# initc3/HoneyBadgerMPC

Measured on AMD Instinct MI355X. Metric: shares reconstructed/sec (batch open, n=64 t=21), higher is better.
Workload: dtype u256 (integer mod p): exact int8 x int8 -> int32 byte-split GEMM on the matrix cores; the high half of every sum folded mod p on the matrix cores too, one-word Barrett quotient

## Files before the change

### honeybadgermpc_amd/_capi.py

```python
import ctypes
import os

import numpy as np

_HERE = os.path.dirname(os.path.abspath(__file__))
LIB_PATH = os.environ.get("HBMPC_HIP_LIB") or os.path.join(_HERE, "lib", "libhbmpc_hip.so")

HB_OK, HB_ERR_SINGULAR, HB_ERR_BAD_ARG, HB_ERR_UNSUPPORTED = 0, 1, 2, 3
HB_ERR_NO_DEVICE, HB_ERR_HIP, HB_ERR_MISMATCH, HB_ERR_RETRY = 4, 5, 6, 7
HB_DEC_COLLECTING, HB_DEC_DONE, HB_DEC_DISAGREE, HB_DEC_UNSUPPORTED, HB_DEC_PENDING = 0, 1, 2, 3, 4
HB_DEC_OPT_DEFER, HB_DEC_OPT_BESIDE = 1, 2
HB_EW_ADD, HB_EW_SUB, HB_EW_MUL, HB_EW_NEG = 0, 1, 2, 3
HB_EW_SELFTEST_BEAVER, HB_EW_SELFTEST_INV, HB_EW_SELFTEST_BROADCAST = 4, 5, 0x100
HB_PM_AUTO, HB_PM_DIRECT, HB_PM_NTT = 0, 1, 2
HB_PM_SELFTEST_SUMS, HB_PM_SELFTEST_POWERS, HB_PM_SELFTEST_TABLES, HB_PM_SELFTEST_MAC, HB_PM_SELFTEST_CONV = 0, 1, 2, 3, 4
HB_BF_SELFTEST_MASK, HB_BF_SELFTEST_SWITCH, HB_BF_SELFTEST_INDEX, HB_BF_SELFTEST_HALVE = 0, 1, 2, 3
HB_MIMC_SUB, HB_MIMC_PAIR = 1, 2
HB_MIMC_SELFTEST_PLAIN, HB_MIMC_SELFTEST_ROUND, HB_MIMC_SELFTEST_FIRST = 0, 1, 2
HB_JJ_SCALAR_BROADCAST, HB_JJ_POINT_BROADCAST = 1, 2
HB_JJ_SELFTEST_SCALAR_MUL, HB_JJ_SELFTEST_DOUBLE_TABLE, HB_JJ_SELFTEST_MASK, HB_JJ_SELFTEST_STAGE1 = 0, 1, 2, 3
HB_JJ_SELFTEST_STAGE2, HB_JJ_SELFTEST_STAGE3, HB_JJ_SELFTEST_SCALE = 4, 5, 6
HB_FXP_MOD, HB_FXP_TRUNC, HB_FXP_NEG_TRUNC = 0, 1, 2
HB_FXP_SELFTEST_MASK, HB_FXP_SELFTEST_TRUNC_PR, HB_FXP_SELFTEST_LEAVES = 0, 1, 2
HB_FXP_SELFTEST_CARRY_MASK, HB_FXP_SELFTEST_CARRY_COMBINE, HB_FXP_SELFTEST_FINISH = 3, 4, 5
# ... 101 lines not shown
    "hb_lt_dmask": (_i, [_vp, _vp, _vp, _vp, _vp, _vp, _i, _vp, _vp, _vp, _vp, _vp, _vp, _i64, _vp]),
    "hb_lt_mid": (_i, [_vp, _vp, _vp, _vp, _i, _vp, _vp, _vp, _vp, _vp, _vp, _vp, _vp, _vp, _vp, _vp, _i64, _vp]),
    "hb_lt_xor_finish": (_i, [_vp, _vp, _vp, _vp, _vp, _vp, _vp, _vp, _i64, _vp]),
    "hb_off_mul_add": (_i, [_vp, _vp, _vp, _vp, _vp, _i64, _vp]),
    "hb_off_invsqrt_scale": (_i, [_vp, _vp, _vp, _i, _vp, _i64, _vp, _vp]),
    "hb_off_degree_check": (_i, [_vp, _vp, _i, _i64, _i, _vp, _vp]),
    "hb_mat_mul": (_i, [_vp, _vp, _vp, _vp, _i, _vp, _i64, _i, _i, _i, _vp]),
    "hb_mat_constants": (_i, [_i, _vp]),
    "hb_quick_interp_check": (_i, [_vp, _vp, _i, _vp, _i, _vp, _i, _vp, _i64, _i64, _i64, _vp, _vp, _vp]),
    "hb_quick_interp_check_map": (_i, [_vp, _vp, _i, _vp, _i, _vp, _i, _vp, _i64, _i64, _i64, _vp, _vp, _vp, _vp]),
    "hb_quick_dec_create": (_i, [_vp, _vp, _i, _pp, _vp]),
    "hb_quick_dec_arrivals": (_i, [_vp, _vp, _i, _i, _i, _vp]),
    "hb_quick_dec_decide": (_i, [_vp, _vp, _i, _vp, _i64, _i64, _i64, _vp, _vp, _vp, _vp]),
    "hb_quick_dec_launch": (_i, [_vp, _vp, _i, _vp, _i64, _i64, _i64, _vp, _vp]),
    "hb_quick_dec_verdict": (_i, [_vp, _vp, _vp]),
    "hb_quick_dec_beside": (_i, [_vp, _i]),
    "hb_quick_dec_destroy": (None, [_vp]),
    "hb_dec_create": (_i, [_vp, _vp, _i, _i, _i, _pp, _vp]),
    "hb_dec_begin": (_i, [_vp, _vp, _i64, _i, _vp, _vp, _i, _vp]),
    "hb_dec_arrived1": (_i, [_vp, _i]),
    "hb_dec_options": (_i, [_vp, _i]),
    "hb_dec_settle": (_i, [_vp]),
    "hb_dec_arrived": (_i, [_vp, _vp, _i, _vp, _vp]),
    "hb_dec_verdict": (_i, [_vp, _vp, _vp]),
    "hb_dec_arrivals_list": (_i, [_vp, _vp, _i, _vp]),
    "hb_dec_destroy": (None, [_vp]),
    "hb_wait_create": (_i, [_vp, _i, _pp]),
    "hb_wait_begin": (_i, [_vp, _vp, _i64, _i64, _i, _i, _i, _i, _vp, _vp, _vp]),
    "hb_wait_arrived1": (_i, [_vp, _i, _i]),
    "hb_wait_result": (_i, [_vp, _i, _vp, _vp, _i, _vp]),
    "hb_wait_destroy": (None, [_vp]),
    "hb_symbols_fetch": (_i, [_vp, _vp, _i, _i64, _i64, _vp, _i, _vp, _vp]),
    "hb_candidate_check": (_i, [_vp, _vp, _i, _vp, _i, _vp, _i64, _i64, _vp, _vp, _vp]),
    "hb_stream_after": (_i, [_vp, _vp, _vp]),
    "hb_side_stream": (_i, [_vp, _pp]),
    "hb_probe_create": (_i, [_vp, _vp, _i, _i, _pp, _vp]),
    "hb_probe_feed": (_i, [_vp, _vp, _i, _vp, _i64, _i64, _i, _vp, _vp, _vp]),
    "hb_probe_reset": (_i, [_vp]),
    "hb_probe_workgroups": (_i, [_vp, _i]),
    "hb_probe_points_fed": (_i, [_vp]),
    "hb_probe_destroy": (None, [_vp]),
    "hb_matvec": (_i, [_vp, _vp, _vp, HbView, _vp, _vp, HbView, _i64, _vp]),
    "hb_matvec_check": (_i, [_vp, _vp, _vp, HbView, _vp, _vp, HbView, _vp, _i, _vp, _i64, _vp]),
    "hb_vandermonde_batch_evaluate": (_i, [_vp, _vp, _i, _vp, _i64, _i, _vp, _vp]),
    "hb_vandermonde_batch_interpolate": (_i, [_vp, _vp, _i, _vp, _i64, _vp, _vp]),
    "hb_fft_batch_evaluate": (_i, [_vp, _vp, _i, _vp, _i64, _i, _i, _vp, _vp]),
    "hb_fft_batch_interpolate": (_i, [_vp, _vp, _i, _vp, _i, _vp, _i64, _vp, _vp]),
    "hb_gao_decode": (_i, [_vp, _vp, _i, _i, _vp, _i64, _vp, _vp, _vp, _vp, _vp]),
    "hb_wb_decode": (_i, [_vp, _vp, _i, _i, _vp, _vp, _i64, _vp, _vp, _vp, _vp]),
    "hb_sqrt_mod": (_i, [_vp, _vp, _i64, _vp, _vp, _vp]),
    "hb_open_plan_create": (_i, [_vp, _i, _i, _i, _vp, _vp, _i, _vp, _vp, _i, _i64, _pp, _vp]),
    "hb_open_r1_encode": (_i, [_vp, _vp, _i64, _vp, _vp]),
    "hb_open_r1_decode": (_i, [_vp, _vp, _i64, _vp, _vp]),
    "hb_open_r2_decode": (_i, [_vp, _vp, _i64, _vp, _vp]),
    "hb_open_status": (_i, [_vp, _vp]),
    "hb_open_plan_set_option": (_i, [_vp, _i, _i]),
    "hb_open_plan_get_option": (_i, [_vp, _i, _vp]),
    "hb_open_plan_destroy": (None, [_vp]),
    "hb_selftest_mulmod": (_i, [_vp, _i, _vp, _vp, _vp]),
    "hb_selftest_ew": (_i, [_vp, _i, _i, _vp, _vp, _i64]),
    "hb_selftest_pm": (_i, [_vp, _i, _i, _vp, _vp, _i64, _i, _i64, _vp]),
    "hb_selftest_bf": (_i, [_vp, _i, _i, _vp, _i64, _i, _vp]),
    "hb_selftest_mimc": (_i, [_vp, _i, _i, _vp, _vp, _i, _i, _i64, _vp, _i64]),
    "hb_selftest_jj": (_i, [_vp, _i, _i, _vp, _vp, _vp, _i, _i64, _vp, _i64]),
    "hb_selftest_fxp": (_i, [_vp, _i, _i, _vp, _vp, _vp, _i64]),
    "hb_selftest_bd": (_i, [_vp, _i, _i, _vp, _vp, _vp, _i64]),
    "hb_selftest_div": (_i, [_vp, _i, _i, _vp, _vp, _vp, _i64]),
    "hb_selftest_eq": (_i, [_vp, _i, _i, _vp, _vp, _vp, _i64]),
    "hb_selftest_lt": (_i, [_vp, _i, _i, _vp, _vp, _vp, _i64]),
    "hb_selftest_off": (_i, [_vp, _i, _i, _vp, _vp, _i64]),
    "hb_selftest_rf": (_i, [_vp, _i, _i, _vp, _vp, _vp]),
    "hb_selftest_mat": (_i, [_vp, _i, _i, _vp, _vp, _vp]),
}
DEBUG_SYMBOLS = {
    "hb_debug_mm8_create": (_i, [_vp, _vp, _i, _i, _pp]),
    "hb_debug_mm8_apply": (_i, [_vp, _vp, _vp, _i64, _i64, _i64, _vp, _i64, _i64, _i64, _i64, _vp, _vp]),
    "hb_debug_occupancy": (_i, [_i, _i, _vp, _vp]),
    "hb_debug_reload_env": (None, []),
    "hb_debug_pm_slab_bytes": (None, [_i64]),
    "hb_debug_rf_stats": (None, [_vp]),
    "hb_debug_rf_profile": (None, [_i]),
    "hb_debug_mat_split": (None, [_i]),
    "hb_debug_matvec_route": (_i, [_vp, _vp, _i64, _vp]),
}

_lib = None


def load_library():
    global _lib
    if _lib is not None:
        return _lib
    import torch

    if torch.cuda.is_available():
        torch.cuda.init()
    if not os.path.exists(LIB_PATH):
        raise HbmpcBackendError(
            f"{LIB_PATH} not found: build it with honeybadgermpc_amd/csrc/build.sh "
            "(or __graft_entry__.build()).  There is no CPU fallback."
        )
    try:
        lib = ctypes.CDLL(LIB_PATH)
    except OSError as e:
        raise HbmpcBackendError(f"cannot load {LIB_PATH}: {e}") from e
    for name, (restype, argtypes) in list(SYMBOLS.items()) + list(DEBUG_SYMBOLS.items()):
        fn = getattr(lib, name)
        fn.restype = restype
        fn.argtypes = argtypes
    _lib = lib
    if _marshal is not None and hasattr(_marshal, "bind_dec"):
        _marshal.bind_dec(ctypes.cast(lib.hb_dec_arrived1, ctypes.c_void_p).value)
        if hasattr(_marshal, "bind_wait"):
            _marshal.bind_wait(ctypes.cast(lib.hb_wait_arrived1, ctypes.c_void_p).value)
    return lib


def _load_marshal():
    try:
        import importlib.util

        path = os.path.join(_HERE, "lib", "_hbmarshal.so")
        spec = importlib.util.spec_from_file_location("_hbmarshal", path)
        mod = importlib.util.module_from_spec(spec)
        spec.loader.exec_module(mod)
        return mod
    except Exception:
        return None


_marshal = _load_marshal()


def ints_to_limbs(values, modulus, nbytes=32):
    if _marshal is not None:
        raw = _marshal.pack(values, modulus, nbytes)
        return np.frombuffer(bytearray(raw), dtype=np.uint64).reshape(len(values), nbytes // 8)
    buf = bytearray(len(values) * nbytes)
    off = 0
    for v in values:
        if v < 0:
            raise OverflowError("can't convert negative int to unsigned")
        if v >= modulus:
            v %= modulus
        buf[off : off + nbytes] = v.to_bytes(nbytes, "little")
        off += nbytes
    return np.frombuffer(buf, dtype=np.uint64).reshape(len(values), nbytes // 8)


def limbs_to_ints(arr, nbytes=32):
    if _marshal is not None:
        return _marshal.unpack(np.ascontiguousarray(arr), nbytes)
    b = np.ascontiguousarray(arr).tobytes()
    return [int.from_bytes(b[i : i + nbytes], "little") for i in range(0, len(b), nbytes)]


def np_ptr(a):
    return a.ctypes.data_as(ctypes.c_void_p)


class Context:

    _cache = {}
    _seen = {}

    @classmethod
# ... 107 lines not shown
```

### honeybadgermpc_amd/csrc/gen_mm8.py

```python
#!/usr/bin/env python3
import os

NC = 47
MAXKB = 4
XB = 180
ABUF = [[196, 200], [204, 208]]
F_SETS = [212, 234]
F_KMIN = -2
CLOBBER_LO, CLOBBER_HI = 180, 255
HALF_RHOS = [(0, 1), (2, 3)]


def f(s, k, e):
    assert -2 <= k <= 8 and e in (0, 1)
    return F_SETS[s] + 2 * (k - F_KMIN) + e


def windows(rho):
    return [q for q in range(-2, 8) if -7 <= 4 * q + rho <= 31]


def cols_of(rho):
    return sorted({4 * q + rho + 7 + 8 * g for q in windows(rho) for g in (0, 1)})


def half_columns(half):
    return sorted(c for rho in HALF_RHOS[half] for c in cols_of(rho))


def lds_loads(kb, xs_op, as_op):
    a0, a1 = ABUF[kb & 1]
    out = []
    for e in (0, 1):
        for h in (0, 1):
            out.append(f"ds_read_b128 v[{XB + 8 * e + 4 * h}:{XB + 8 * e + 4 * h + 3}], {xs_op} offset:{((kb * 2 + e) * 2 + h) * 1024}")
    out.append(f"ds_read_b128 v[{a0}:{a0 + 3}], {as_op} offset:{(kb * 2) * 1024}")
    out.append(f"ds_read_b128 v[{a1}:{a1 + 3}], {as_op} offset:{(kb * 2 + 1) * 1024}")
    return out


def interleave(mfmas, ops):
    out = []
    if not mfmas:
        return list(ops)
    n = len(mfmas)
    per = (len(ops) + max(n - 1, 1) - 1) // max(n - 1, 1)
    pi = 0
    for i, m in enumerate(mfmas):
        if i == n - 1:
            out += ops[pi:]
            pi = len(ops)
        out.append(m)
        if i < n - 1:
            out += ops[pi:pi + per]
            pi += per
    return out


def asm_half(half, nkb, skip=False):
    assert not skip or nkb >= 2
    cols = half_columns(half)
    pos = {c: i for i, c in enumerate(cols)}
    ncol = len(cols)
    xs_op, as_op, bias = f"%{ncol}", f"%{ncol + 1}", f"%{ncol + 2}"
    L = []
    for s in range(2):
        for k in (-2, 8):
            for e in (0, 1):
                L.append(f"v_mov_b32 v{f(s, k, e)}, 0")
    L += lds_loads(0, xs_op, as_op)[:(5 if skip else 6)]
    groups = [(kb, rho) for kb in range(nkb) for rho in HALF_RHOS[half]]

    def prep(gi):
        kb, rho = groups[gi]
        s = gi & 1
        ops = []
        if rho == HALF_RHOS[half][0]:
            ops.append("s_waitcnt lgkmcnt(0)")
            for e in (0, 1):
                for k in range(8):
                    ops.append(f"v_xor_b32 v{f(s, k, e)}, 0x80808080, v{XB + 8 * e + k}")
                ops.append(f"v_mov_b32 v{f(s, -1, e)}, 0")
            if rho != 0:
                for e in (0, 1):
                    for k in range(-1, 8):
                        ops.append(f"v_alignbyte_b32 v{f(s, k, e)}, v{f(s, k + 1, e)}, v{f(s, k, e)}, {rho}")
        else:
            for e in (0, 1):
                for k in range(-1, 8):
                    ops.append(f"v_alignbyte_b32 v{f(s, k, e)}, v{f(1 - s, k + 1, e)}, v{f(1 - s, k, e)}, 1")
        return ops

    started = set()

    def mfmas(gi):
        kb, rho = groups[gi]
        s = gi & 1
        out = []
        for q in windows(rho):
            r = f(s, q, 0)
            assert r % 2 == 0
            for grp in (0, 1):
                if skip and kb == 0 and grp == 1:
                    continue
                c = 4 * q + rho + 7 + 8 * grp
                ab = ABUF[kb & 1][grp]
                cin = f"%{pos[c]}"
                if c not in started:
                    assert kb == 0 or (skip and kb == 1)
                    cin = bias
                    started.add(c)
                out.append(f"v_mfma_i32_16x16x64_i8 %{pos[c]}, v[{ab}:{ab + 3}], v[{r}:{r + 3}], {cin}")
        return out

    L += prep(0) + ["s_nop 1"]
    for gi in range(len(groups)):
        nxt = gi + 1 < len(groups)
        kb, rho = groups[gi]
        if rho == HALF_RHOS[half][0] and kb + 1 < nkb:
            L += lds_loads(kb + 1, xs_op, as_op)
        L += interleave(mfmas(gi), prep(gi + 1) if nxt else [])
        if nxt:
            L.append("s_nop 0")
    assert started == set(cols)
    L += ["s_nop 7", "s_nop 7"]
    return L, ncol


def emit():
    out = ["// GENERATED by gen_mm8.py -- do not edit", ""]
    out.append("// column held by accumulator i of each half (half 0: rho in {0,1}; half 1: rho in {2,3})")
    for half in range(2):
        cols = half_columns(half)
        out.append(f"// half {half}: {cols}")
    assert half_columns(0) == [c for c in range(NC) if c % 4 in (0, 3)] and half_columns(1) == [c for c in range(NC) if c % 4 in (1, 2)]
    out.append("template <int NKB, int HALF, bool SKIP = false> struct Mm8Phase;")
    clob = ", ".join(f'"v{r}"' for r in range(CLOBBER_LO, CLOBBER_HI + 1))
    for nkb, skip in [(k, False) for k in range(1, MAXKB + 1)] + [(k, True) for k in range(2, MAXKB + 1)]:
        for half in range(2):
            lines, ncol = asm_half(half, nkb, skip)
            out.append(f"template <> struct Mm8Phase<{nkb}, {half}, {'true' if skip else 'false'}> {{")
            out.append("    static __device__ __forceinline__ void run(v4i (&acc)[24], uint32_t xs_addr, uint32_t as_addr, v4i biasv) {")
            out.append("        asm volatile(")
            for ln in lines:
                out.append(f'            "{ln}\\n\\t"')
            outs = ", ".join(f'"=&v"(acc[{i}])' for i in range(ncol))
            out.append(f"            : {outs}")
            out.append('            : "v"(xs_addr), "v"(as_addr), "v"(biasv)')
            out.append(f'            : {clob}, "memory");')
            out.append("    }")
            out.append("};")
    return "\n".join(out) + "\n"


if __name__ == "__main__":
    here = os.path.dirname(os.path.abspath(__file__))
    text = emit()
    path = os.path.join(here, "hb_mm8_body.inc")
    old = open(path).read() if os.path.exists(path) else None
    if old != text:
        open(path, "w").write(text)
    print(path)
```

### honeybadgermpc_amd/csrc/hb_common.hpp

```cpp
#pragma once
#include <hip/hip_runtime.h>
#include <stdint.h>
#include <stdio.h>
#include <string.h>

#include <functional>
#include <map>
#include <mutex>
#include <string>
#include <vector>

#include "../../include/hbmpc_hip.h"
#include "fp29.hpp"

namespace hb {
struct FastMatrix;
struct Mm8Matrix;
struct Mm8wMatrix;
}
namespace hb {

struct Wide { static constexpr int NL = 9, NW = 8; };
struct Narrow { static constexpr int NL = 3, NW = 2; };

constexpr int OT = 4;

template <int NL, int NW>
__device__ __forceinline__ void eval_at_point_128(uint32_t (&r)[NL], const uint32_t *__restrict__ x_packed, const uint32_t *__restrict__ poly, int d,
                                                  const FpParams<NL> &P, uint32_t (*red)[NL]) {
    const int tid = threadIdx.x;
    uint32_t xd[NL], xm[NL], acc[NL];
    load_digits<NL, NW>(xd, x_packed);
    to_mont(xm, xd, P);
#pragma unroll
    for (int q = 0; q < NL; q++) acc[q] = 0;
    for (int l = tid; l < d; l += 128) {
        uint32_t pw[NL], cd[NL], m[NL];
        fp_pow_u32(pw, xm, (uint32_t)l, P);
        load_digits<NL, NW>(cd, poly + (size_t)l * NW);
        mont_mul(m, cd, pw, P);
        fp_add(acc, acc, m, P);
    }
#pragma unroll
    for (int q = 0; q < NL; q++) red[tid][q] = acc[q];
    __syncthreads();
    for (int w = 64; w >= 1; w >>= 1) {
        if (tid < w) {
            uint32_t a[NL], b[NL], t[NL];
#pragma unroll
            for (int q = 0; q < NL; q++) { a[q] = red[tid][q]; b[q] = red[tid + w][q]; }
            fp_add(t, a, b, P);
#pragma unroll
            for (int q = 0; q < NL; q++) red[tid][q] = t[q];
        }
        __syncthreads();
    }
#pragma unroll
    for (int q = 0; q < NL; q++) r[q] = red[0][q];
}

__host__ __device__ inline size_t m_index(int i, int l, int n_in, int nl, int q) {
    return (((size_t)((i / OT) * n_in + l) * (size_t)nl + (size_t)q) * OT) + (size_t)(i % OT);
}
inline int m_tiles(int n_out) { return (n_out + OT - 1) / OT; }

}

struct hb_matrix {
    hb_ctx *ctx;
    int n_out, n_in;
    uint32_t *dev;
    size_t words;
    bool cached;
    int refs;
    hb::Mm8wMatrix *wide;
    bool wide_tried;
};

namespace hb {
struct TlsError {
    static std::string &slot() { static thread_local std::string s; return s; }
    TlsError &operator=(const std::string &m) { slot() = m; return *this; }
    TlsError &operator=(const char *m) { slot() = m ? m : ""; return *this; }
    const char *c_str() const { return slot().c_str(); }
    void clear() { slot().clear(); }
    bool empty() const { return slot().empty(); }
};
struct PrescaleParams {
    uint32_t pbar[9];
    uint32_t pneg[8];
    uint32_t m0, m1;
};
}
namespace hb {
enum EnvHook {
    ENV_CACHE_CAP,
    ENV_GAO_PAIR,
    ENV_MM8W_FLAT,
    ENV_MM8W_RQ,
    ENV_MM8W_TILE16,
    ENV_MM8_NO_SKIP,
    ENV_NO_EVAL_FEW,
    ENV_NO_FUSED_SMALL,
    ENV_NO_FUSED_VALIDATE,
    ENV_NO_MFMA,
    ENV_NO_MFMA_DECODE,
    ENV_NO_MFMA_WIDE,
    ENV_NO_NARROW_FAST,
    ENV_NO_QUICK,
    ENV_NO_QUICK_PLAN,
    ENV_NTT_STAGE_LOOP,
    ENV_PROBE_WGS,
    ENV_QUICK_NO_CAND,
    ENV_UPLOAD_MODE,
    ENV_WB_NO_GAO,
    ENV_WB_NO_UNIFORM,
    ENV_COUNT
};
const char *env_hook(EnvHook h);
void env_reload();
}
struct hb_ctx {
    int device;
    int n_limbs;
    hb::FpParams<9> pw;
    hb::FpParams<3> pn;
    uint64_t p_limbs[4];
    std::recursive_mutex mu;
    int api_depth = 0;
    hb::TlsError err;
    std::map<std::string, hb_matrix *> mcache;
    std::map<std::vector<int32_t>, int32_t *> icache;
    std::map<std::string, void *> dcache;
    std::map<std::string, hb::FastMatrix *> fcache;
    std::map<std::string, hb::Mm8Matrix *> m8cache;
    struct CacheSlot { uint64_t tick; bool pinned; std::function<void()> drop; };
    std::map<std::string, CacheSlot> lru;
    uint64_t lru_clock = 0;
    size_t cache_cap = 192;
    int32_t *flag_dev;
    hb::PrescaleParams psc;
    int psc_state = 0;
    std::map<std::string, void *> ptcache;
    struct QuickSlot { void *buf = nullptr; size_t cap = 0; void *ev = nullptr; };
    std::vector<QuickSlot> qslots;
    unsigned qnext = 0;
    std::vector<void *> probe_pool, probe_host_pool;
    void *side_stream = nullptr;
    std::map<std::string, std::pair<void *, size_t>> scratch;
    void *fetch_host = nullptr, *fetch_dev = nullptr;
    int fetch_seq = 0;
    void *cand_host = nullptr, *cand_dev = nullptr;
    int32_t *cand_ticket = nullptr;
    int cand_seq = 0;
    void *after_event = nullptr;
    std::map<int, void *> wide_shared;
    std::map<std::string, std::vector<int>> wide_shapes;
    void *mm8_shared = nullptr;
    int elem_words() const { return n_limbs == 4 ? 8 : 2; }
    int nl() const { return n_limbs == 4 ? 9 : 3; }
};

struct hb_api_guard {
    hb_ctx *c;
    explicit hb_api_guard(hb_ctx *ctx) : c(ctx) { if (c) { c->mu.lock(); c->api_depth++; } }
    ~hb_api_guard() { if (c) { c->api_depth--; c->mu.unlock(); } }
    hb_api_guard(const hb_api_guard &) = delete;
    hb_api_guard &operator=(const hb_api_guard &) = delete;
};
#define HB_API_GUARD(ctxexpr) hb_api_guard hb_api_guard__(ctxexpr)

inline int ctx_scratch(hb_ctx *ctx, const char *slot, size_t bytes, void **out) {
    auto &e = ctx->scratch[slot];
    if (e.second < bytes || !e.first) {
        if (e.first) { (void)hipFree(e.first); e.first = nullptr; e.second = 0; }
        const size_t want = bytes ? bytes : 4;
        const hipError_t err = hipMalloc(&e.first, want);
        if (err != hipSuccess) { e.first = nullptr; ctx->err = std::string("scratch ") + slot + ": " + hipGetErrorString(err); return HB_ERR_HIP; }
        e.second = want;
    }
    *out = e.first;
    return HB_OK;
}
inline void ctx_scratch_free(hb_ctx *ctx) {
    for (auto &kv : ctx->scratch) if (kv.second.first) (void)hipFree(kv.second.first);
// ... 85 lines not shown
                   int64_t C, hipStream_t s, int check_skip = 0, const uint32_t *K_override = nullptr);

int launch_decode_check(hb_ctx *ctx, const FastMatrix *dec, const FastMatrix *enc, const uint32_t *cols, hb_view cv,
                        const int32_t *z_dev, uint32_t *pk_dst, hb_view pv, int64_t pk_count, int pk_rows, uint32_t *coef_dg,
                        const int32_t *mask_dev, int32_t *mismatch_dev, int64_t C, hipStream_t s, int check_skip);

bool prescale_params(hb_ctx *ctx);
int mm8_from_fast(hb_ctx *ctx, const FastMatrix *f, Mm8Matrix **out, hipStream_t s, const int32_t *rows = nullptr, int n_rows = 0);
void mm8_free(Mm8Matrix *m);
int launch_mm8(hb_ctx *ctx, const Mm8Matrix *m, const uint32_t *in, hb_view iv, const int32_t *in_rows_dev, int64_t in_count,
               uint32_t *out, hb_view ov, int64_t out_count, const int32_t *check_mask_dev, int32_t *mismatch_dev,
               int64_t C, hipStream_t s, uint32_t *copy_dst = nullptr, hb_view cpv = hb_view{0, 0}, int64_t copy_count = 0,
               int copy_rows = 0, const int32_t *check_rows_dev = nullptr);

int mm8w_from_host(hb_ctx *ctx, const uint64_t *m_host, int n_out, int n_in, Mm8wMatrix **out, hipStream_t s);
void mm8w_free(Mm8wMatrix *m);
int mm8w_route(hb_ctx *ctx, const Mm8wMatrix *m, int64_t C, int32_t *out);
int launch_mm8w(hb_ctx *ctx, const Mm8wMatrix *m, const uint32_t *in, hb_view iv, const int32_t *in_rows_dev, int64_t in_count,
                uint32_t *out, hb_view ov, int64_t out_count, const int32_t *check_mask_dev, int32_t *mismatch_dev,
                int64_t C, hipStream_t s, const uint32_t *cmp = nullptr, hb_view cv = hb_view{0, 0}, int n_store = 0);
bool fold_tables(hb_ctx *ctx, int n_bytes, uint8_t *fold, uint32_t *top8, uint32_t *mu, uint32_t *shift8);
struct FsVerdict { unsigned long long word; unsigned long long pad; };
struct FsDone { int32_t *counter; FsVerdict *host; int32_t seq; };
constexpr int32_t FS_VERDICT_NONE = 0x3fffffff;
#ifdef __HIPCC__
__device__ __forceinline__ void fs_publish_verdict(int32_t *mismatch, int32_t *first_bad, int32_t *counter, FsVerdict *host, int32_t seq) {
    const int32_t fl = mismatch ? __hip_atomic_load(mismatch, __ATOMIC_RELAXED, __HIP_MEMORY_SCOPE_AGENT) : 0;
    const int32_t fb = first_bad ? __hip_atomic_load(first_bad, __ATOMIC_RELAXED, __HIP_MEMORY_SCOPE_AGENT) : INT32_MAX;
    const uint32_t low = ((fl & 1) ? 0x80000000u : 0u) | ((fl & 0x40000000) ? 0x40000000u : 0u) | (uint32_t)((fb < 0 || fb > FS_VERDICT_NONE) ? FS_VERDICT_NONE : fb);
    __hip_atomic_store(&host->word, ((unsigned long long)(uint32_t)seq << 32) | low, __ATOMIC_RELAXED, __HIP_MEMORY_SCOPE_SYSTEM);
    if (mismatch) __hip_atomic_store(mismatch, 0, __ATOMIC_RELAXED, __HIP_MEMORY_SCOPE_AGENT);
    if (first_bad) __hip_atomic_store(first_bad, INT32_MAX, __ATOMIC_RELAXED, __HIP_MEMORY_SCOPE_AGENT);
    if (counter) __hip_atomic_store(counter, 0, __ATOMIC_RELAXED, __HIP_MEMORY_SCOPE_AGENT);
}
__device__ __forceinline__ void fs_workgroup_done(const FsDone &done, int32_t *mismatch, int32_t *first_bad) {
    if (!done.counter) return;
    asm volatile("s_waitcnt vmcnt(0)" ::: "memory");
    __syncthreads();
    if (threadIdx.x == 0 && atomicAdd(done.counter, 1) == (int)gridDim.x - 1) fs_publish_verdict(mismatch, first_bad, done.counter, done.host, done.seq);
}
#endif
inline bool fs_verdict_is(const FsVerdict *host, int32_t seq) { return (int32_t)(*reinterpret_cast<const volatile unsigned long long *>(&host->word) >> 32) == seq; }
inline void fs_verdict_read(const FsVerdict *host, int32_t *flag, int32_t *first) {
    const uint32_t low = (uint32_t)*reinterpret_cast<const volatile unsigned long long *>(&host->word);
    *flag = ((low >> 31) ? 1 : 0) | ((low & 0x40000000u) ? 0x40000000 : 0);
    const int32_t f = (int32_t)(low & 0x3fffffffu);
    *first = f == FS_VERDICT_NONE ? INT32_MAX : f;
}
struct Mm8wShared { uint32_t bias; uint32_t c80r[9], biasmod[9]; void *wp; uint32_t *zero; };
int mm8w_geometry(int n_out, int d, int *tile_rows, int *n_rt, int *nkb, size_t *a8_bytes, size_t *crow_words);
int mm8w_shared(hb_ctx *ctx, int d, const Mm8wShared **out, hipStream_t s);
void mm8w_shared_free(hb_ctx *ctx);
int launch_mm8w_raw(hb_ctx *ctx, int n_out, int d, int tile_rows, const void *a8, const uint32_t *crow, const Mm8wShared *sh,
                    const uint32_t *in, hb_view iv, const int32_t *in_rows_dev, int64_t in_count, uint32_t *out, hb_view ov, int64_t out_count,
                    const int32_t *check_mask_dev, int32_t *mismatch_dev, int64_t C, hipStream_t s, const uint32_t *cmp, hb_view cv, int n_store,
                    int32_t *first_bad_dev, uint32_t *bad_map_dev = nullptr, const FsDone *done = nullptr);
void point_tables_free(hb_ctx *ctx);
void mm8_shared_free(hb_ctx *ctx);
struct PointTable {
    int n, S;
    uint32_t *xm, *inv, *pw;
    bool usable;
    int refs;
    bool small;
    std::vector<uint16_t> xs;
    uint16_t *xs_dev;
};
int point_table(hb_ctx *ctx, const uint64_t *x_host, int n, PointTable **out, hipStream_t s);
struct QuickLayout {
    int n, d, nc, n_coef, n_out, tile_rows, nkb;
    size_t o_a8, o_crow, o_wj, o_full, o_nraw, o_mcan, o_z, o_map, o_sync, need;
    size_t o_cand, o_cand_crow;
};
int quick_layout(hb_ctx *ctx, int n, int d, int nc, int n_coef, QuickLayout *L);
int quick_build(hb_ctx *ctx, const uint64_t *x_host, const int32_t *z, const int32_t *zc, const QuickLayout &L, uint8_t *base, const Mm8wShared **shared, hipStream_t s,
                int flags = 3 );
int quick_layout_cand(hb_ctx *ctx, QuickLayout *L);
int quick_launch(hb_ctx *ctx, const QuickLayout &L, const uint8_t *base, const Mm8wShared *sh, const uint32_t *cols, hb_view cv, uint32_t *out, hb_view ov,
                 int64_t out_count, int n_store, int32_t *mismatch_dev, int32_t *first_bad_dev, int64_t C, hipStream_t s, uint32_t *bad_map_dev = nullptr,
                 const FsDone *done = nullptr);
struct FsLayout {
    int n, d, nc, n_coef, n_out, n_rt, nkb;
    size_t o_a8, o_crow, o_kt, o_mode, o_z, o_cand, o_cand_crow, need;
};
constexpr int FS_BUILD_Z = 1, FS_BUILD_ZC = 2;
int fs_layout(hb_ctx *ctx, const PointTable *pt, int d, int nc, int n_coef, FsLayout *L);
int fs_build(hb_ctx *ctx, const PointTable *pt, const int32_t *z, const int32_t *zc, const FsLayout &L, uint8_t *base, int flags, int32_t *status_dev, hipStream_t s);
int fs_launch(hb_ctx *ctx, const FsLayout &L, const uint8_t *base, const uint32_t *cols, hb_view cv, uint32_t *out, hb_view ov, int64_t out_count,
              int32_t *mismatch_dev, int32_t *first_bad_dev, uint32_t *bad_map_dev, int64_t C, hipStream_t s, const FsDone *done = nullptr,
              const int32_t *pick_zc = nullptr);
int fs_build_cand(hb_ctx *ctx, PointTable *pt, const int32_t *z, const FsLayout &L, uint8_t *base, int32_t *status_dev, hipStream_t s, bool with_z = false);
struct Mv64Matrix;
int points_on_device(hb_ctx *ctx, const uint64_t *x_host, int n, uint32_t **out, hipStream_t s);
bool mv64_applies(const hb_ctx *ctx, int d);
bool mv64_matrix_cores(const hb_ctx *ctx, int d);
int mv64_from_host(hb_ctx *ctx, const uint64_t *m_host, int n_out, int d, const int32_t *mode_host, Mv64Matrix **out, hipStream_t s);
void mv64_free(Mv64Matrix *m);
int launch_mv64(hb_ctx *ctx, const Mv64Matrix *m, const uint64_t *in, hb_view iv, const int32_t *in_rows_dev, int64_t in_count, uint64_t *out, hb_view ov,
                int64_t out_count, int32_t *mismatch_dev, int32_t *first_bad_dev, int64_t C, hipStream_t s);
int mv64_plan_tables(hb_ctx *ctx, const uint64_t *x, int n, int d, const int32_t *z, const int32_t *zc, int nc, std::vector<uint64_t> &V, std::vector<uint64_t> &Vinv,
                     std::vector<uint64_t> &P);
int quick_dec_supported(hb_quick_dec *qd, int d, int nc, int n_coef);
const Mm8wMatrix *matrix_wide(hb_ctx *ctx, const hb_matrix *m, hipStream_t s);

#define HB_DISPATCH(ctx, EXPR_W, EXPR_N)                                                          \
    do {                                                                                          \
        if ((ctx)->n_limbs == 4) { EXPR_W; } else { EXPR_N; }                                     \
    } while (0)

}
```

### honeybadgermpc_amd/csrc/hb_core.hip

```cpp
#include <algorithm>

#include <mutex>
#include <string>

#include "hb_common.hpp"

using namespace hb;

namespace {

struct U320 { uint64_t l[5]; };
inline bool ge(const U320 &a, const U320 &b) {
    for (int i = 4; i >= 0; i--) if (a.l[i] != b.l[i]) return a.l[i] > b.l[i];
    return true;
}
inline void sub(U320 &a, const U320 &b) {
    unsigned __int128 br = 0;
    for (int i = 0; i < 5; i++) {
        unsigned __int128 d = (unsigned __int128)a.l[i] - b.l[i] - (uint64_t)br;
        a.l[i] = (uint64_t)d; br = (d >> 64) & 1;
    }
}
inline void dbl_mod(U320 &a, const U320 &p) {
    for (int i = 4; i > 0; i--) a.l[i] = (a.l[i] << 1) | (a.l[i - 1] >> 63);
// ... 342 lines not shown
    return HB_OK;
}

int alloc_matrix(hb_ctx *ctx, int n_out, int n_in, hb_matrix **out) {
    hb_matrix *m = new hb_matrix();
    m->ctx = ctx; m->n_out = n_out; m->n_in = n_in; m->cached = false; m->refs = 1; m->wide = nullptr; m->wide_tried = false;
    m->words = (size_t)m_tiles(n_out) * (size_t)n_in * OT * (size_t)ctx->nl();
    if (m->words == 0) m->words = 1;
    hipError_t e = hipMalloc(&m->dev, m->words * sizeof(uint32_t));
    if (e != hipSuccess) { delete m; ctx->err = std::string("hipMalloc: ") + hipGetErrorString(e); return HB_ERR_HIP; }
    *out = m;
    return HB_OK;
}

__global__ void k_upload_copy(const uint4 *__restrict__ src, uint4 *__restrict__ dst, size_t n16) {
    const size_t i = (size_t)blockIdx.x * blockDim.x + threadIdx.x;
    if (i < n16) dst[i] = src[i];
}
int upload_table(hb_ctx *ctx, void *dst_dev, const void *src_host, size_t bytes, hipStream_t s) {
    if (bytes == 0) return HB_OK;
    static const int legacy = [] { const char *e = env_hook(ENV_UPLOAD_MODE); return e && !strcmp(e, "memcpy") ? 1 : 0; }();
    if (legacy) {
        hipError_t e = hipMemcpyAsync(dst_dev, src_host, bytes, hipMemcpyHostToDevice, s);
        if (e == hipSuccess) e = hipStreamSynchronize(s);
        if (e != hipSuccess) { ctx->err = std::string("table upload: ") + hipGetErrorString(e); return HB_ERR_HIP; }
        return HB_OK;
    }
    const size_t n16 = (bytes + 15) / 16;
    void *stage = nullptr;
    HB_HIP(ctx, hipMalloc(&stage, n16 * 16));
    hipError_t e = hipMemcpy(stage, src_host, bytes, hipMemcpyHostToDevice);
    if (e == hipSuccess) {
        if (bytes % 16 == 0) k_upload_copy<<<(unsigned)((n16 + 255) / 256), 256, 0, s>>>((const uint4 *)stage, (uint4 *)dst_dev, n16);
        else e = hipMemcpyAsync(dst_dev, stage, bytes, hipMemcpyDeviceToDevice, s);
    }
    if (e == hipSuccess) e = hipGetLastError();
    if (e == hipSuccess) e = hipStreamSynchronize(s);
    (void)hipFree(stage);
    if (e != hipSuccess) { ctx->err = std::string("table upload: ") + hipGetErrorString(e); return HB_ERR_HIP; }
    return HB_OK;
}

int upload_elems(hb_ctx *ctx, const uint64_t *host, size_t count, uint32_t **dev, hipStream_t s) {
    size_t bytes = count * (size_t)ctx->elem_words() * 4;
    HB_HIP(ctx, hipMalloc(dev, bytes ? bytes : 4));
    const int rc = upload_table(ctx, *dev, host, bytes, s);
    if (rc) { (void)hipFree(*dev); *dev = nullptr; }
    return rc;
}

int points_on_device(hb_ctx *ctx, const uint64_t *x_host, int n, uint32_t **out, hipStream_t s) {
    std::string key = table_key("xs", ctx, x_host, n, 0);
    auto it = ctx->dcache.find(key);
    if (it != ctx->dcache.end()) { *out = (uint32_t *)it->second; cache_touch(ctx, "d|" + key); return HB_OK; }
    uint32_t *xd = nullptr;
    const int rc = upload_elems(ctx, x_host, (size_t)n, &xd, s); if (rc) return rc;
    ctx->dcache[key] = xd;
    cache_note(ctx, "d|" + key, [ctx, key]() { auto f = ctx->dcache.find(key); if (f != ctx->dcache.end()) { (void)hipFree(f->second); ctx->dcache.erase(f); } });
    *out = xd;
    return HB_OK;
}

std::string table_key(const char *kind, hb_ctx *ctx, const uint64_t *x, int n, int d) {
    std::string k(kind);
    k += ":" + std::to_string(n) + ":" + std::to_string(d) + ":";
    k.append(reinterpret_cast<const char *>(x), (size_t)n * ctx->n_limbs * 8);
    return k;
}

}

template <int NL, int NW>
__global__ void __launch_bounds__(128) k_eval_few(const FpParams<NL> P, const uint32_t *__restrict__ x, int n, const uint32_t *__restrict__ polys, int d,
                                                  uint32_t *__restrict__ out) {
    __shared__ uint32_t red[128][NL];
    const int c = blockIdx.x / n, i = blockIdx.x - c * n;
    uint32_t r[NL];
    eval_at_point_128<NL, NW>(r, x + (size_t)i * NW, polys + (size_t)c * d * NW, d, P, red);
    if (threadIdx.x == 0) store_digits<NL, NW>(out + ((size_t)c * n + i) * NW, r);
}


namespace hb {
static const char *const ENV_NAMES[ENV_COUNT] = {"HB_CACHE_CAP", "HB_GAO_PAIR", "HB_MM8W_FLAT", "HB_MM8W_RQ", "HB_MM8W_TILE16", "HB_MM8_NO_SKIP", "HB_NO_EVAL_FEW", "HB_NO_FUSED_SMALL", "HB_NO_FUSED_VALIDATE", "HB_NO_MFMA", "HB_NO_MFMA_DECODE", "HB_NO_MFMA_WIDE", "HB_NO_NARROW_FAST", "HB_NO_QUICK", "HB_NO_QUICK_PLAN", "HB_NTT_STAGE_LOOP", "HB_PROBE_WGS", "HB_QUICK_NO_CAND", "HB_UPLOAD_MODE", "HB_WB_NO_GAO", "HB_WB_NO_UNIFORM"};
static std::string g_env_val[ENV_COUNT];
static bool g_env_set[ENV_COUNT];
static std::once_flag g_env_once;
static std::mutex g_env_mu;
static void env_read() {
    for (int i = 0; i < ENV_COUNT; i++) {
        const char *e = ::getenv(ENV_NAMES[i]);
        g_env_set[i] = e != nullptr;
        g_env_val[i] = e ? e : "";
    }
}
const char *env_hook(EnvHook h) {
    std::call_once(g_env_once, env_read);
    return g_env_set[h] ? g_env_val[h].c_str() : nullptr;
}
void env_reload() {
    std::call_once(g_env_once, env_read);
    std::lock_guard<std::mutex> lk(g_env_mu);
    env_read();
}
}
extern "C" void hb_debug_reload_env() { hb::env_reload(); }

extern "C" {

int hb_version(void) { return 100; }

int hb_device_count(void) {
    int n = 0;
    if (hipGetDeviceCount(&n) != hipSuccess) return 0;
    return n;
}

int hb_ctx_create(hb_ctx **out, const uint64_t *p_limbs, int n_limbs, int device) {
    if (!out || !p_limbs) return HB_ERR_BAD_ARG;
    *out = nullptr;
    if (n_limbs != 1 && n_limbs != 4) return HB_ERR_BAD_ARG;
    if ((p_limbs[0] & 1) == 0) return HB_ERR_UNSUPPORTED;
    bool small = true; for (int i = 1; i < n_limbs; i++) if (p_limbs[i]) small = false;
    if (small && p_limbs[0] < 3) return HB_ERR_UNSUPPORTED;
    int ndev = 0;
    if (hipGetDeviceCount(&ndev) != hipSuccess || ndev == 0) return HB_ERR_NO_DEVICE;
    if (device < 0 || device >= ndev) return HB_ERR_NO_DEVICE;
    if (hipSetDevice(device) != hipSuccess) return HB_ERR_NO_DEVICE;
    hb_ctx *ctx = new hb_ctx();
    ctx->device = device; ctx->n_limbs = n_limbs;
    memset(ctx->p_limbs, 0, sizeof ctx->p_limbs);
    memcpy(ctx->p_limbs, p_limbs, (size_t)n_limbs * 8);
    if (n_limbs == 4) make_params<9>(ctx->pw, p_limbs, 4); else make_params<3>(ctx->pn, p_limbs, 1);
    if (const char *e = env_hook(ENV_CACHE_CAP)) { long v = atol(e); if (v >= 1) ctx->cache_cap = (size_t)v; }
    ctx->flag_dev = nullptr;
    if (hipMalloc(&ctx->flag_dev, 64 * sizeof(int32_t)) != hipSuccess) { delete ctx; return HB_ERR_HIP; }
    (void)hipMemset(ctx->flag_dev, 0, 64 * sizeof(int32_t));
    *out = ctx;
    return HB_OK;
}

void hb_ctx_destroy(hb_ctx *ctx) {
    if (!ctx) return;
    (void)hipSetDevice(ctx->device);
    ctx->lru.clear();
    for (auto &kv : ctx->mcache) matrix_unref(kv.second);
    for (auto &kv : ctx->icache) (void)hipFree(kv.second);
    for (auto &kv : ctx->dcache) (void)hipFree(kv.second);
    for (auto &kv : ctx->fcache) fast_matrix_free(kv.second);
    for (auto &kv : ctx->m8cache) mm8_free(kv.second);
    if (ctx->flag_dev) (void)hipFree(ctx->flag_dev);
    if (ctx->side_stream) (void)hipStreamDestroy((hipStream_t)ctx->side_stream);
    point_tables_free(ctx);
    mm8w_shared_free(ctx);
    mm8_shared_free(ctx);
    ctx_scratch_free(ctx);
    delete ctx;
}

const char *hb_last_error(const hb_ctx *ctx) { return ctx ? ctx->err.c_str() : "no context"; }
int hb_elem_bytes(const hb_ctx *ctx) { return ctx ? ctx->n_limbs * 8 : 0; }

int hb_malloc(hb_ctx *ctx, void **dptr, size_t bytes) { HB_API_GUARD(ctx); HB_HIP(ctx, hipMalloc(dptr, bytes ? bytes : 4)); return HB_OK; }
int hb_free(hb_ctx *ctx, void *dptr) { HB_API_GUARD(ctx); HB_HIP(ctx, hipFree(dptr)); return HB_OK; }
int hb_memcpy_h2d(hb_ctx *ctx, void *dst, const void *src, size_t bytes, void *stream) { HB_API_GUARD(ctx);
    HB_HIP(ctx, hipMemcpyAsync(dst, src, bytes, hipMemcpyHostToDevice, (hipStream_t)stream)); return HB_OK;
}
// ... 439 lines not shown
```

### honeybadgermpc_amd/csrc/hb_mfma.hip

```cpp
#include <atomic>

#include "hb_mm8.hpp"

namespace hb {

#include "hb_mm8_body.inc"

#ifdef HB_MM8_TIMING
__device__ unsigned long long g_mm8_t[2048 * 8];
#define MM8_T(k) do { const unsigned long long tn_ = __builtin_amdgcn_s_memtime(); tacc[k] += tn_ - tlast; tlast = tn_; } while (0)
#else
#define MM8_T(k) do { } while (0)
#endif
template <int NKB, bool CHECK, bool RAGGED, bool SKIP>
__global__ __launch_bounds__(256, 2) void k_mm8(const int4 *__restrict__ a8, const uint32_t *__restrict__ crowd,
                                                const uint32_t *__restrict__ zero_src,
                                                const uint32_t *__restrict__ in_pk, int64_t in_sc, int64_t in_sl,
                                                const int32_t *__restrict__ in_rows, int64_t in_count, int d,
                                                uint32_t *__restrict__ out_pk, int64_t out_sc, int64_t out_sl, int64_t out_count,
                                                const int32_t *__restrict__ check_mask, const int32_t *__restrict__ check_rows, int32_t *__restrict__ mismatch,
                                                uint32_t *__restrict__ copy_dst, int64_t copy_sc, int64_t copy_sl, int64_t copy_count, int copy_rows,
                                                int n_out, int n_rt, int tpw, int64_t n_chunks, int64_t n_units, BarrettParams bp) {
    extern __shared__ uint4 mm8_lds[];
    const int lane = threadIdx.x & 63, wave = __builtin_amdgcn_readfirstlane(threadIdx.x >> 6);
// ... 317 lines not shown
Big big_divmod(const Big &x, const Big &p, Big *q) {
    Big r(p.size() + 1, 0), pp(p); pp.push_back(0);
    if (q) q->assign(x.size(), 0);
    for (int bit = (int)x.size() * 32 - 1; bit >= 0; bit--) {
        uint32_t in = (x[bit >> 5] >> (bit & 31)) & 1u;
        for (size_t i = r.size(); i-- > 0;) r[i] = (r[i] << 1) | (i ? r[i - 1] >> 31 : in);
        if (big_ge(r, pp)) { big_sub(r, pp); if (q) (*q)[bit >> 5] |= 1u << (bit & 31); }
    }
    r.pop_back();
    return r;
}
Big big_shl(const Big &a, int bits, size_t words) {
    Big r(words, 0);
    for (size_t i = 0; i < a.size(); i++) {
        const size_t w = i + bits / 32; const int s = bits % 32;
        if (w < words) r[w] |= a[i] << s;
        if (s && w + 1 < words) r[w + 1] |= a[i] >> (32 - s);
    }
    return r;
}

}

namespace hb {

bool prescale_params(hb_ctx *ctx) {
    if (ctx->psc_state) return ctx->psc_state > 0;
    ctx->psc_state = -1;
    if (ctx->n_limbs != 4 || (ctx->p_limbs[3] >> 62) == 0) return false;
    Big p(8);
    for (int i = 0; i < 4; i++) { p[2 * i] = (uint32_t)ctx->p_limbs[i]; p[2 * i + 1] = (uint32_t)(ctx->p_limbs[i] >> 32); }
    Big pw9(p); pw9.push_back(0);
    Big pb(9, 0); pb[8] = 1u << 5;
    big_sub(pb, pw9);
    for (int k = 0; k < 9; k++) {
        const int bit = 29 * k, j = bit >> 5, sft = bit & 31;
        const uint64_t v = pb[j] | ((uint64_t)(j + 1 < 9 ? pb[j + 1] : 0) << 32);
        ctx->psc.pbar[k] = (uint32_t)(v >> sft) & DMASK;
    }
    Big pn(9, 0); pn[8] = 1;
    big_sub(pn, pw9);
    for (int k = 0; k < 8; k++) ctx->psc.pneg[k] = pn[k];
    Big two290(10, 0); two290[9] = 1u << 2;
    Big mu; big_divmod(two290, p, &mu);
    const uint64_t muv = mu[0] | ((uint64_t)mu[1] << 32);
    ctx->psc.m0 = (uint32_t)muv & DMASK;
    ctx->psc.m1 = (uint32_t)(muv >> LB);
    ctx->psc_state = 1;
    return true;
}

void mm8_free(Mm8Matrix *m) {
    if (!m) return;
    (void)hipFree(m->a8); (void)hipFree(m->crow); (void)hipFree(m->zero);
    delete m;
}

int mm8_shared(hb_ctx *ctx, const Mm8Shared **out, hipStream_t s) {
    if (ctx->mm8_shared) { *out = static_cast<const Mm8Shared *>(ctx->mm8_shared); return HB_OK; }
    if (ctx->n_limbs != 4 || (ctx->p_limbs[3] >> 62) == 0 || !prescale_params(ctx)) return fail(ctx, HB_ERR_UNSUPPORTED, "mm8: modulus");
    Mm8Shared *sh = new Mm8Shared();
    memset(sh, 0, sizeof *sh);
    Big p(8);
    for (int k = 0; k < 4; k++) { p[2 * k] = (uint32_t)ctx->p_limbs[k]; p[2 * k + 1] = (uint32_t)(ctx->p_limbs[k] >> 32); }
    uint32_t shift8[8];
    if (!fold_tables(ctx, 16, sh->fold_host, sh->bp.c384, &sh->bp.mu, shift8)) { delete sh; return fail(ctx, HB_ERR_UNSUPPORTED, "mm8: fold table"); }
    {
        Big pn(9, 0); pn[8] = 1;
        Big pw9(p); pw9.push_back(0);
        big_sub(pn, pw9);
        for (int k = 0; k < 8; k++) sh->bp.pneg[k] = pn[k];
    }
    auto digits9 = [](const Big &v, uint32_t *dg) {
        for (int k = 0; k < 9; k++) {
            const int bit = 29 * k, j = bit >> 5, sft = bit & 31;
            const uint64_t w = (uint64_t)(j < (int)v.size() ? v[j] : 0) | ((uint64_t)(j + 1 < (int)v.size() ? v[j + 1] : 0) << 32);
            dg[k] = (uint32_t)(w >> sft) & DMASK;
        }
    };
    Big biasmod;
    { Big bt(14, 0); for (int c = 0; c < MM8_NC; c++) { Big t(1, (uint32_t)MM8_BIAS); big_add(bt, big_shl(t, 8 * c, 14)); } biasmod = big_divmod(bt, p, nullptr); }
    { Big sft(shift8, shift8 + 8); if (!big_ge(biasmod, sft)) big_add(biasmod, p); big_sub(biasmod, sft); }
    digits9(biasmod, sh->biasmod);
    {
        Big c80(8, 0x80808080u);
        Big r261(9, 0); r261[8] = 1u << 5;
        digits9(big_divmod(big_mul(c80, r261), p, nullptr), sh->c80r);
    }
    if (hipMalloc(&sh->fold_dev, sizeof sh->fold_host) != hipSuccess) { delete sh; return fail(ctx, HB_ERR_HIP, "mm8: hipMalloc(fold table)"); }
    if (int rc = upload_table(ctx, sh->fold_dev, sh->fold_host, sizeof sh->fold_host, s)) { (void)hipFree(sh->fold_dev); delete sh; return rc; }
    ctx->mm8_shared = sh;
    *out = sh;
    return HB_OK;
}

void mm8_shared_free(hb_ctx *ctx) {
    Mm8Shared *sh = static_cast<Mm8Shared *>(ctx->mm8_shared);
    if (!sh) return;
    (void)hipFree(sh->fold_dev);
    delete sh;
    ctx->mm8_shared = nullptr;
}

int mm8_from_fast(hb_ctx *ctx, const FastMatrix *f, Mm8Matrix **out, hipStream_t s, const int32_t *rows, int n_rows) {
    *out = nullptr;
    if (env_hook(ENV_NO_MFMA)) return HB_ERR_UNSUPPORTED;
    if (ctx->n_limbs != 4 || f->n_in < 1 || f->n_in > 32 || f->n_out < 1) return HB_ERR_UNSUPPORTED;
    if ((ctx->p_limbs[3] >> 62) == 0) return HB_ERR_UNSUPPORTED;
    const int n_out = rows ? n_rows : f->n_out, d = f->n_in, nkb = (d + 7) / 8, n_rt = (n_out + 15) / 16;
    if (n_out < 1) return HB_ERR_UNSUPPORTED;
    if (mm8_lds_bytes(n_rt, nkb, (n_rt == 1) ? 4 : (n_rt == 2) ? 2 : 1) > MM8_LDS_LIMIT) return HB_ERR_UNSUPPORTED;
    const int tiles = (f->n_out + f->ot - 1) / f->ot;
    std::vector<uint32_t> Mh((size_t)tiles * d * f->ot * 9);
    std::vector<int32_t> neg((size_t)f->n_out, 0);
    HB_HIP(ctx, hipMemcpyAsync(Mh.data(), f->M, Mh.size() * 4, hipMemcpyDeviceToHost, s));
    if (f->negrow) HB_HIP(ctx, hipMemcpyAsync(neg.data(), f->negrow, neg.size() * 4, hipMemcpyDeviceToHost, s));
    HB_HIP(ctx, hipStreamSynchronize(s));

    Big p(8);
    for (int k = 0; k < 4; k++) { p[2 * k] = (uint32_t)ctx->p_limbs[k]; p[2 * k + 1] = (uint32_t)(ctx->p_limbs[k] >> 32); }
    Big c80(8, 0x80808080u);
    c80 = big_divmod(c80, p, nullptr);
    Big biasmod;
    { Big bt(14, 0); for (int c = 0; c < MM8_NC; c++) { Big t(1, (uint32_t)MM8_BIAS); big_add(bt, big_shl(t, 8 * c, 14)); } biasmod = big_divmod(bt, p, nullptr); }
    std::vector<uint8_t> foldtab((size_t)MM8_FOLD_Q * 16, 0);
    BarrettParams bpar;
    {
        uint32_t shift8[8];
        if (!fold_tables(ctx, 16, foldtab.data(), bpar.c384, &bpar.mu, shift8)) return HB_ERR_UNSUPPORTED;
        Big sh(shift8, shift8 + 8);
        if (!big_ge(biasmod, sh)) big_add(biasmod, p);
        big_sub(biasmod, sh);
    }

    std::vector<int8_t> a((size_t)n_rt * nkb * 2 * 64 * 16, 0);
    bool skip01 = nkb >= 2 && !env_hook(ENV_MM8_NO_SKIP);
    std::vector<uint32_t> cr((size_t)n_rt * 16 * 16 + (size_t)MM8_FOLD_Q * 4, 0);
    memcpy(&cr[(size_t)n_rt * 16 * 16], foldtab.data(), foldtab.size());
    for (size_t i = 0; i < (size_t)n_rt * 16; i++) for (int k = 0; k < 8; k++) { cr[i * 16 + 2 * k] = 0x10100000u; cr[i * 16 + 2 * k + 1] = 0x1010u; }
    for (int i = 0; i < n_out; i++) {
        Big pos(5, 0), ngs(5, 0);
        int64_t colsum = 0;
        const int src = rows ? rows[i] : i;
        if (src < 0 || src >= f->n_out) return HB_ERR_BAD_ARG;
        for (int l = 0; l < d; l++) {
            uint32_t dg[9], w8[8];
            for (int q = 0; q < 9; q++) dg[q] = Mh[mf_index(src, l, d, 9, q, f->ot)];
            pack<9, 8>(w8, dg);
            if (w8[4] | w8[5] | w8[6] | w8[7]) return HB_ERR_UNSUPPORTED;
            const int sgn = neg[src] ? -1 : 1;
            int carry = 0;
            const int lane_ = (4 * ((i % 16) % 4) + (i % 16) / 4) + 16 * ((l % 8) / 2), el = l & 1;
            for (int b = 0; b < 16; b++) {
                int t = sgn * (int)((w8[b >> 2] >> (8 * (b & 3))) & 0xffu) + carry;
                if (t > 127) { t -= 256; carry = 1; } else if (t < -128) { t += 256; carry = -1; } else carry = 0;
                const int grp = b >> 3, r7 = 7 - (b & 7), hi = r7 >> 2, bi = r7 & 3;
                a[((((size_t)(i / 16) * nkb + l / 8) * 2 + grp) * 64 + (size_t)lane_) * 16 + 4 * (2 * hi + el) + bi] = (int8_t)t;
                if (t != 0 && grp == 1 && l < 8) skip01 = false;
                colsum += (t < 0) ? -t : t;
            }
            if (carry) return HB_ERR_UNSUPPORTED;
            Big e(w8, w8 + 4);
            big_add(neg[src] ? ngs : pos, e);
        }
        if (colsum * 128 > MM8_BIAS) return HB_ERR_UNSUPPORTED;
        Big cp = big_divmod(big_mul(c80, pos), p, nullptr), cn = big_divmod(big_mul(c80, ngs), p, nullptr);
// ... 105 lines not shown
```

### honeybadgermpc_amd/csrc/hb_mfma_fused.hip

```cpp
#include <math.h>

#include <algorithm>
#include <atomic>
#include <type_traits>

#include "hb_mm8.hpp"

namespace hb {

#include "hb_mm8_body.inc"

constexpr int FS_WAVES = 8, FS_TPW = 4;
#ifdef HB_MM8_TIMING
__device__ unsigned long long g_fs_t[256 * 8 * 8];
#define FS_T(k) do { const unsigned long long tn_ = __builtin_amdgcn_s_memtime(); tacc[k] += tn_ - tlast; tlast = tn_; } while (0)
#else
#define FS_T(k) do { } while (0)
#endif
constexpr int FS_MAXD = 24, FS_MAXC = 104;
constexpr size_t FS_LDS_LIMIT = 156 * 1024;

struct FsIdx { uint16_t z[FS_MAXD], xz[FS_MAXD], zc[FS_MAXC], xzc[FS_MAXC]; };
struct FsPick { const uint4 *cand; const uint32_t *cand_crow; int n_coef, nc; uint16_t zc[FS_MAXC]; };
struct FsSplit { uint32_t terms[FS_WAVES]; };
constexpr int FS_CAND_MAXN = 128;

__host__ __device__ inline size_t fs_lds_bytes(int n_rt, int nkb) {
    return ((size_t)n_rt * 64 + (size_t)n_rt * nkb * 2 * 64 + (size_t)2 * FS_TPW * nkb * 4 * 64 + MM8_FOLD_Q) * 16 + (size_t)(32 + 16 * n_rt) * 4;
}

template <int NKB>
__global__ __launch_bounds__(64 * FS_WAVES, 2) void k_mm8f(const int4 *__restrict__ a8, const uint32_t *__restrict__ crowd, const v4i *__restrict__ foldg,
                                                          const uint32_t *__restrict__ KT, const PrescaleParams PP,
                                                          const uint32_t *__restrict__ in_pk, int64_t in_sc, int64_t in_sl, const int32_t *__restrict__ in_rows,
                                                          int64_t in_count, int d, const int32_t *__restrict__ rowmode,
                                                          uint32_t *__restrict__ out_pk, int64_t out_sc, int64_t out_sl, int64_t out_count,
                                                          int32_t *__restrict__ mismatch, int32_t *__restrict__ first_bad, uint32_t *__restrict__ bad_map,
                                                          int n_out, int n_rt, int64_t n_chunks, int64_t n_units, BarrettParams bp, const FsDone done, const FsPick pick,
                                                          const FsSplit split) {
    constexpr int NT = 64 * FS_WAVES, NL = 9, NW = 8;
    extern __shared__ uint4 fs_lds[];
    const int lane = threadIdx.x & 63, wave = __builtin_amdgcn_readfirstlane(threadIdx.x >> 6);
    const int n = lane & 15, g = lane >> 4;
    uint32_t *crl = reinterpret_cast<uint32_t *>(fs_lds);
    int4 *abuf = reinterpret_cast<int4 *>(fs_lds + n_rt * 64);
    uint4 *xbuf = fs_lds + n_rt * 64 + n_rt * NKB * 2 * 64;
    constexpr int bufsz = FS_TPW * NKB * 4 * 64;
    int32_t *rowl = reinterpret_cast<int32_t *>(xbuf + 2 * bufsz);
    int32_t *maskl = rowl + 32;
    v4i *foldl = reinterpret_cast<v4i *>(maskl + 16 * n_rt);

#ifdef HB_MM8_TIMING
    unsigned long long tacc[8] = {0, 0, 0, 0, 0, 0, 0, 0}, tlast = __builtin_amdgcn_s_memtime();
#endif
    auto unit_chunk = [&](int64_t unit) {
        const int64_t chunk = unit * 64 + lane;
        return chunk >= n_chunks ? n_chunks - 1 : chunk;
    };
    auto fetch_row = [&](int64_t chunk, int row, uint32_t (&w)[NW], bool &okk) {
        const int64_t idx = chunk * in_sc + (int64_t)row * in_sl;
        okk = idx < in_count;
        load_words<NW>(w, in_pk + (okk ? idx : 0) * NW);
    };
    const uint32_t first_terms = (0x01010101u << wave) & (d < 32 ? (1u << d) - 1u : ~0u);
    uint32_t x_first[NW] = {0, 0, 0, 0, 0, 0, 0, 0};
    bool ok_first = false;
    if (first_terms) {
        const int l0 = __builtin_ctz(first_terms);
        fetch_row(unit_chunk(blockIdx.x), in_rows ? in_rows[l0] : l0, x_first, ok_first);
    }
    uint4 pk_piece = make_uint4(0, 0, 0, 0), pk_crow = make_uint4(0, 0, 0, 0);
    const int pk_e = threadIdx.x;
    const bool pk_has_piece = pick.cand && pk_e < pick.nc * NKB * 8, pk_has_crow = pick.cand && pk_e < pick.nc * 4;
    if (pk_has_piece) {
        const int j = pk_e / (NKB * 8), pc = pk_e - j * (NKB * 8);
        pk_piece = pick.cand[(size_t)pick.zc[j] * (NKB * 8) + pc];
    }
    if (pk_has_crow) pk_crow = reinterpret_cast<const uint4 *>(pick.cand_crow)[(size_t)pick.zc[pk_e >> 2] * 4 + (pk_e & 3)];
    {
        const int tid = threadIdx.x, n_mask = n_rt * 16, n_crow = n_rt * 64, n_img = n_rt * NKB * 2 * 64;
        const int lc = tid < d ? tid : d - 1;
        int32_t rw = in_rows ? in_rows[lc] : lc;
        int32_t mk = rowmode[tid < n_out ? tid : 0];
        v4i cr = reinterpret_cast<const v4i *>(crowd)[tid < n_crow ? tid : 0];
        v4i fo = foldg[tid < MM8_FOLD_Q ? tid : 0];
        v4i img[3];
#pragma unroll
        for (int k = 0; k < 3; k++) img[k] = reinterpret_cast<const v4i *>(a8)[tid + k * NT < n_img ? tid + k * NT : 0];
        asm volatile("" : "+v"(rw), "+v"(mk), "+v"(cr), "+v"(fo), "+v"(img[0]), "+v"(img[1]), "+v"(img[2]));
        if (tid < 32) rowl[tid] = rw;
        if (tid < n_mask) maskl[tid] = tid < n_out ? mk : 0;
        if (tid < n_crow) reinterpret_cast<v4i *>(fs_lds)[tid] = cr;
        if (tid < MM8_FOLD_Q) foldl[tid] = fo;
#pragma unroll
        for (int k = 0; k < 3; k++)
            if (tid + k * NT < n_img) reinterpret_cast<v4i *>(abuf)[tid + k * NT] = img[k];
        for (int i = tid + NT; i < n_mask; i += NT) maskl[i] = i < n_out ? rowmode[i] : 0;
        for (int i = tid + NT; i < n_crow; i += NT) fs_lds[i] = reinterpret_cast<const uint4 *>(crowd)[i];
        for (int i = tid + 3 * NT; i < n_img; i += NT) abuf[i] = a8[i];
    }
    for (int i = threadIdx.x; i < (8 * NKB - d) * 256; i += NT) {
        const int l = d + (i >> 8), b = (i >> 7) & 1, t = (i >> 5) & 3, h = (i >> 4) & 1, c = i & 15;
        const int kb = l >> 3, gg = (l & 7) >> 1, e = l & 1;
        xbuf[(size_t)b * bufsz + (size_t)((((t * NKB + kb) * 2 + e) * 2 + h) * 64) + (c + 16 * gg)] = make_uint4(0, 0, 0, 0);
    }
    const int n_pairs = FS_TPW * n_rt;
    const uint32_t my_terms = (uint32_t)__builtin_amdgcn_readfirstlane((int)split.terms[wave]);

    auto scale_unit = [&](auto first, int64_t unit, uint4 *dst, uint32_t terms) {
        constexpr bool FIRST = decltype(first)::value;
        const int64_t chunk = unit_chunk(unit);
        const int t = lane >> 4;
        uint32_t xw[NW];
        bool ok = false;
        auto fetch = [&](int l, uint32_t (&w)[NW], bool &okk) { fetch_row(chunk, FIRST ? (in_rows ? in_rows[l] : l) : rowl[l], w, okk); };
        terms &= d < 32 ? (1u << d) - 1u : ~0u;
        int l = terms ? __builtin_ctz(terms) : d;
        if constexpr (FIRST) {
#pragma unroll
            for (int k = 0; k < NW; k++) xw[k] = x_first[k];
            ok = ok_first;
        } else if (l < d) fetch(l, xw, ok);
        while (l < d) {
            terms &= terms - 1u;
            const int ln = terms ? __builtin_ctz(terms) : d;
            uint32_t xn[NW];
            bool okn = false;
            fetch(ln < d ? ln : l, xn, okn);
            const uint32_t *__restrict__ T = KT + (size_t)l * (NL * NL);
            uint32_t xd[NL];
            unpack<NL, NW>(xd, xw);
            uint64_t col[NL + 1];
#pragma unroll
            for (int j = 0; j <= NL; j++) col[j] = 0;
#pragma unroll
            for (int q = 0; q < NL; q++)
#pragma unroll
                for (int j = 0; j < NL; j++) col[j] += (uint64_t)xd[q] * T[q * NL + j];
            uint32_t v[NL + 1];
#pragma unroll
            for (int k = 0; k < NL; k++) { v[k] = (uint32_t)col[k] & DMASK; col[k + 1] += col[k] >> LB; }
            v[NL] = (uint32_t)col[NL];
            const uint64_t mid = (uint64_t)v[9] * PP.m0 + (uint64_t)v[8] * PP.m1 + (((uint64_t)v[8] * PP.m0) >> LB);
            const uint64_t qh = (uint64_t)v[9] * PP.m1 + (mid >> LB);
            const uint32_t q0 = (uint32_t)qh & DMASK, q1 = (uint32_t)(qh >> LB);
            uint64_t dc[NL];
#pragma unroll
            for (int k = 0; k < NL; k++) {
                dc[k] = v[k] + (uint64_t)q0 * PP.pbar[k];
                if (k > 0) dc[k] += (uint64_t)q1 * PP.pbar[k - 1];
            }
            uint32_t r[NL];
#pragma unroll
            for (int k = 0; k < NL; k++) {
                r[k] = (uint32_t)dc[k] & DMASK;
                if (k < NL - 1) dc[k + 1] += dc[k] >> LB;
            }
            uint32_t w[NW];
            pack<NL, NW>(w, r);
            if (PP.pneg[NW - 1] >> 31) {
#pragma unroll
                for (int k = 0; k < NW; k++) w[k] = ok ? w[k] : 0u;
            } else {
                uint32_t u[NW];
                unsigned cy = 0;
#pragma unroll
                for (int k = 0; k < NW; k++) u[k] = __builtin_addc(w[k], PP.pneg[k], cy, &cy);
                const bool take = cy || (r[NL - 1] >> 24);
#pragma unroll
                for (int k = 0; k < NW; k++) w[k] = ok ? (take ? u[k] : w[k]) : 0u;
            }
            const int kb = l >> 3, gg = (l & 7) >> 1, e = l & 1;
            uint4 *slot = dst + (size_t)(((t * NKB + kb) * 2 + e) * 2) * 64 + (n + 16 * gg);
            slot[0] = make_uint4(w[0], w[1], w[2], w[3]);
            slot[64] = make_uint4(w[4], w[5], w[6], w[7]);
#pragma unroll
            for (int k = 0; k < NW; k++) xw[k] = xn[k];
            ok = okn;
            l = ln;
        }
    };

    scale_unit(std::true_type{}, blockIdx.x, xbuf, first_terms);
    if (pick.cand) {
        __syncthreads();
        auto put = [&](int e, const uint4 &v) {
            const int j = e / (NKB * 8), pc = e - j * (NKB * 8);
            const int ri = pick.n_coef + j, rt = ri >> 4, r16 = ri & 15, r = 4 * (r16 & 3) + (r16 >> 2);
            const int kb = pc >> 3, grp = (pc >> 2) & 1, gg = pc & 3;
            reinterpret_cast<uint4 *>(abuf)[((rt * NKB + kb) * 2 + grp) * 64 + r + 16 * gg] = v;
        };
        if (pk_has_piece) put(pk_e, pk_piece);
        for (int e = pk_e + NT; e < pick.nc * NKB * 8; e += NT) {
            const int j = e / (NKB * 8), pc = e - j * (NKB * 8);
            put(e, pick.cand[(size_t)pick.zc[j] * (NKB * 8) + pc]);
        }
        if (pk_has_crow) fs_lds[(pick.n_coef + (pk_e >> 2)) * 4 + (pk_e & 3)] = pk_crow;
        for (int j = threadIdx.x; j < pick.nc; j += NT) maskl[pick.n_coef + j] = (int32_t)pick.zc[j] + 1;
    }

    const v4i biasv = v4i{MM8_BIAS, MM8_BIAS, MM8_BIAS, MM8_BIAS};
    uint32_t k256 = 256u, k16m = 1u << 24;
    int32_t s1 = 1, s256 = 256, s64k = 1 << 16, s16m = 1 << 24;
    uint32_t u1 = 1u;
    asm volatile("" : "+s"(k256), "+s"(k16m), "+s"(s1), "+s"(s256), "+s"(s64k), "+s"(s16m), "+s"(u1));
    const v4i *fold_lane = reinterpret_cast<const v4i *>(reinterpret_cast<const char *>(foldl) + (g == (n >> 2) ? 16 * n : 256));

    int buf = 0;
    int64_t unit = blockIdx.x;
    FS_T(0);
    for (; unit < n_units; unit += gridDim.x, buf ^= 1) {
        asm volatile("s_waitcnt lgkmcnt(0)" ::: "memory");
        FS_T(7);
        __builtin_amdgcn_s_barrier();
        FS_T(1);
        if (my_terms && unit + gridDim.x < n_units) scale_unit(std::false_type{}, unit + gridDim.x, xbuf + (size_t)(buf ^ 1) * bufsz, my_terms);
        FS_T(2);
        for (int pidx = wave; pidx < n_pairs; pidx += FS_WAVES) {
            const int tl = n_rt == 2 ? (pidx >> 1) : pidx / n_rt;
            const int rt = n_rt == 2 ? ((pidx ^ (pidx >> 2)) & 1) : pidx - tl * n_rt;
            const int64_t chunk = (unit * FS_TPW + tl) * 16 + n;
            const uint4 *xs = xbuf + (size_t)buf * bufsz + (size_t)tl * NKB * 4 * 64 + lane;
            const int4 *as = abuf + (size_t)rt * NKB * 2 * 64 + lane;
            uint32_t eap[4][11], c0p[4];
            const int rows_here = n_out - 16 * rt < 16 ? n_out - 16 * rt : 16;
            const int nreg = (rows_here + 3) >> 2;
            const uint32_t xs_addr = (uint32_t)(uintptr_t)(__attribute__((address_space(3))) const void *)xs;
            const uint32_t as_addr = (uint32_t)(uintptr_t)(__attribute__((address_space(3))) const void *)as;
            {
                v4i acc[24];
                asm volatile("" ::: "memory");
                __builtin_amdgcn_sched_barrier(0);
                __builtin_amdgcn_s_setprio(0);
                Mm8Phase<NKB, 0, false>::run(acc, xs_addr, as_addr, biasv);
                __builtin_amdgcn_s_setprio(2);
                __builtin_amdgcn_sched_barrier(0);
                FS_T(3);
#pragma unroll
                for (int reg = 0; reg < 4; reg++) {
                    if (reg >= 2 && reg >= nreg) break;
                    c0p[reg] = (uint32_t)acc[0][reg];
#pragma unroll
                    for (int j = 0; j < 11; j++) eap[reg][j] = (uint32_t)acc[1 + 2 * j][reg] + ((uint32_t)acc[2 + 2 * j][reg] << 8);
                    asm volatile("" ::"v"(c0p[reg]), "v"(eap[reg][0]), "v"(eap[reg][1]), "v"(eap[reg][2]), "v"(eap[reg][3]), "v"(eap[reg][4]),
                                 "v"(eap[reg][5]), "v"(eap[reg][6]), "v"(eap[reg][7]), "v"(eap[reg][8]), "v"(eap[reg][9]), "v"(eap[reg][10]));
                    __builtin_amdgcn_sched_barrier(0);
                }
            }
            {
                v4i acc[24];
                asm volatile("" ::: "memory");
                __builtin_amdgcn_sched_barrier(0);
                FS_T(4);
                __builtin_amdgcn_s_setprio(0);
                Mm8Phase<NKB, 1, false>::run(acc, xs_addr, as_addr, biasv);
                __builtin_amdgcn_s_setprio(2);
                __builtin_amdgcn_sched_barrier(0);
                FS_T(5);
#pragma unroll
                for (int reg = 0; reg < 4; reg++) {
                    if (reg >= 2 && reg >= nreg) break;
                    const int i = 16 * rt + 4 * reg + g;
                    const int md = maskl[i];
                    const bool live = chunk < n_chunks;
                    const bool cmp = live && md > 0, st = live && md < 0;
                    uint32_t ew[8];
                    load_words<8>(ew, in_pk + (cmp ? (chunk * in_sc + (int64_t)(md - 1) * in_sl) * 8 : 0));
                    uint64_t pw[8];
                    {
                        const uint4 *cr = reinterpret_cast<const uint4 *>(crl + (size_t)i * 16);
#pragma unroll
                        for (int k = 0; k < 4; k++) {
                            const uint4 c = cr[k];
                            pw[2 * k] = (uint64_t)c.x | ((uint64_t)c.y << 32);
                            pw[2 * k + 1] = (uint64_t)c.z | ((uint64_t)c.w << 32);
                        }
                    }
                    uint32_t glo[5], ghi[5];
#pragma unroll
                    for (int k = 0; k < 12; k++) {
                        const uint32_t f = (uint32_t)acc[2 * k][reg] + ((uint32_t)acc[2 * k + 1][reg] << 8);
                        uint64_t gk = (uint64_t)f * k256 + (k < 7 ? pw[k] : 0ull);
                        if (k < 11) gk += (uint64_t)eap[reg][k] * k16m;
                        if (k < 7) pw[k] = gk;
                        else { glo[k - 7] = (uint32_t)gk; ghi[k - 7] = (uint32_t)(gk >> 32); }
                    }
                    pw[0] += (uint64_t)c0p[reg] * u1;
                    pw[7] += (uint64_t)glo[0] * u1;
                    uint32_t hw[5];
                    {
                        unsigned cyw = 0;
#pragma unroll
                        for (int k = 0; k < 4; k++) hw[k] = __builtin_addc(glo[k + 1], ghi[k], cyw, &cyw);
                        hw[4] = ghi[4] + cyw;
                    }
                    v4i hb;
#pragma unroll
                    for (int k = 0; k < 4; k++) hb[k] = (int)(hw[k] ^ 0x80808080u);
                    v4i dcol[8];
#pragma unroll
                    for (int eb = 0; eb < 8; eb++)
                        dcol[eb] = __builtin_amdgcn_mfma_i32_16x16x64_i8(fold_lane[eb * (MM8_FOLD_ROW / 16)], hb, v4i{0, 0, 0, 0}, 0, 0, 0);
#pragma unroll
                    for (int k = 0; k < 8; k++) pw[k] += (uint64_t)hw[4] * bp.c384[k];
#pragma unroll
                    for (int k = 0; k < 8; k++) {
                        int64_t tt = (int64_t)pw[k] + (int64_t)dcol[k][0] * s1;
                        tt += (int64_t)dcol[k][1] * s256;
                        tt += (int64_t)dcol[k][2] * s64k;
                        tt += (int64_t)dcol[k][3] * s16m;
                        pw[k] = (uint64_t)tt;
                    }
                    const uint64_t tq = pw[7] + (pw[6] >> 32);
                    const uint32_t qh = (uint32_t)(((uint64_t)(uint32_t)(tq >> 16) * bp.mu) >> 46);
#pragma unroll
                    for (int k = 0; k < 8; k++) pw[k] += (uint64_t)qh * bp.pneg[k];
                    uint32_t ow[8];
                    uint32_t top;
                    {
                        unsigned cy = 0;
                        ow[0] = (uint32_t)pw[0];
#pragma unroll
                        for (int k = 1; k < 8; k++) ow[k] = __builtin_addc((uint32_t)pw[k], (uint32_t)(pw[k - 1] >> 32), cy, &cy);
                        top = (uint32_t)(pw[7] >> 32) + cy - qh;
                    }
                    if (__builtin_amdgcn_ballot_w64(top != 0 || ow[7] >= ~bp.pneg[7]) != 0) {
                        uint32_t u[8];
                        unsigned cy2 = 0;
#pragma unroll
                        for (int k = 0; k < 8; k++) u[k] = __builtin_addc(ow[k], bp.pneg[k], cy2, &cy2);
                        const bool take = cy2 || top;
#pragma unroll
                        for (int k = 0; k < 8; k++) ow[k] = take ? u[k] : ow[k];
                    }
                    uint32_t diff = 0;
#pragma unroll
                    for (int k = 0; k < 8; k++) diff |= ew[k] ^ ow[k];
                    asm volatile("" : "+v"(diff), "+v"(ow[0]), "+v"(ow[1]), "+v"(ow[2]), "+v"(ow[3]), "+v"(ow[4]), "+v"(ow[5]), "+v"(ow[6]), "+v"(ow[7]));
                    const unsigned long long bad_lanes = __builtin_amdgcn_ballot_w64(cmp && diff);
                    if (bad_lanes) {
                        const uint32_t bits16 = (uint32_t)((bad_lanes | (bad_lanes >> 16) | (bad_lanes >> 32) | (bad_lanes >> 48)) & 0xffffull);
                        if (lane == 0) {
                            const int64_t tile_base = chunk - n;
                            const int32_t cmin = (int32_t)tile_base + __builtin_ctz(bits16);
                            if (*reinterpret_cast<volatile int32_t *>(mismatch) == 0) atomicOr(mismatch, 1);
                            if (first_bad && *reinterpret_cast<volatile int32_t *>(first_bad) > cmin) atomicMin(first_bad, cmin);
                            if (bad_map) atomicOr(bad_map + (tile_base >> 5), bits16 << (tile_base & 31));
                        }
                    }
                    const int64_t oidx = chunk * out_sc + (int64_t)(-md - 1) * out_sl;
                    if (st && oidx < out_count) store_words<8>(out_pk + oidx * 8, ow);
                    if (reg & 1) __builtin_amdgcn_sched_barrier(0);
                }
            }
            FS_T(6);
        }
    }
#ifdef HB_MM8_TIMING
    if (lane == 0 && blockIdx.x < 256) for (int k = 0; k < 8; k++) g_fs_t[(blockIdx.x * 8 + wave) * 8 + k] = tacc[k];
#endif
    fs_workgroup_done(done, mismatch, first_bad);
}

typedef __int128 i128;

struct FsConsts { uint32_t c80r[9], biasmod[9]; };
constexpr int32_t FS_OVERFLOW = 0x40000000;

__device__ __forceinline__ size_t fs_digit_addr(int i, int l, int b, int nkb) {
    const int lane_ = (4 * ((i % 16) % 4) + (i % 16) / 4) + 16 * ((l % 8) / 2), el = l & 1;
    const int grp = b >> 3, r7 = 7 - (b & 7), hi = r7 >> 2, bi = r7 & 3;
    return ((((size_t)(i / 16) * nkb + l / 8) * 2 + grp) * 64 + (size_t)lane_) * 16 + 4 * (2 * hi + el) + bi;
}

__device__ __forceinline__ void fs_row_constant(const FpParams<9> &P, const FsConsts &cs, const i128 *row, int d, uint32_t *dst16) {
    constexpr int NL = 9, NW = 8;
    uint32_t s5[5] = {0, 0, 0, 0, 0};
    for (int l = 0; l < d; l++) {
        const i128 v = row[l];
        const uint32_t vw[5] = {(uint32_t)v, (uint32_t)(v >> 32), (uint32_t)(v >> 64), (uint32_t)(v >> 96), (uint32_t)(v >> 127 >> 1)};
        unsigned cy = 0;
#pragma unroll
        for (int k = 0; k < 5; k++) s5[k] = __builtin_addc(s5[k], vw[k], cy, &cy);
    }
    const bool negs = (s5[4] >> 31) != 0;
    if (negs) {
        unsigned cy = 1;
#pragma unroll
        for (int k = 0; k < 5; k++) s5[k] = __builtin_addc(~s5[k], 0u, cy, &cy);
    }
    uint32_t w8[NW] = {s5[0], s5[1], s5[2], s5[3], s5[4], 0, 0, 0}, fe[NL], prod[NL], corr[NL], k80[NL], bm[NL];
    unpack<NL, NW>(fe, w8);
    if (negs) fp_neg(fe, fe, P);
#pragma unroll
    for (int k = 0; k < NL; k++) { k80[k] = cs.c80r[k]; bm[k] = cs.biasmod[k]; }
    mont_mul(prod, fe, k80, P);
    fp_sub(corr, prod, bm, P);
    uint32_t cw[NW];
    pack<NL, NW>(cw, corr);
#pragma unroll
    for (int k = 0; k < 8; k++) {
        const uint64_t pair = (uint64_t)cw[k] + ((0x1010ull << 32) | 0x10100000ull);
        dst16[2 * k] = (uint32_t)pair;
        dst16[2 * k + 1] = (uint32_t)(pair >> 32);
    }
}

__device__ __forceinline__ void fs_build_body(uint8_t *fb_lds, const FpParams<9> &P, const uint32_t *__restrict__ inv, int n, const FsIdx &ix, int d, int nc, int n_coef,
                                              int flags, const FsConsts &cs, uint8_t *__restrict__ a8, uint32_t *__restrict__ crow, uint32_t *__restrict__ KT,
                                              int32_t *__restrict__ rowmode, int32_t *__restrict__ z_dev, int32_t *__restrict__ status) {
    constexpr int NL = 9, NW = 8;
    const int n_out = n_coef + nc, nkb = (d + 7) / 8, n_rt = (n_out + 15) / 16;
    i128 *ent = reinterpret_cast<i128 *>(fb_lds);
    i128 *Ac = ent + (size_t)n_out * d;
    uint32_t *wj = reinterpret_cast<uint32_t *>(Ac + (d + 1));
    uint32_t *part = wj + (size_t)d * NL;
    const int tid = threadIdx.x;
    const bool do_z = flags & FS_BUILD_Z, do_zc = flags & FS_BUILD_ZC;
    if (do_z) {
        const size_t img = (size_t)n_rt * nkb * 2 * 64 * 16;
        for (size_t i = tid; i < img / 16; i += 1024) reinterpret_cast<uint4 *>(a8)[i] = make_uint4(0, 0, 0, 0);
        for (int i = tid; i < n_rt * 16 * 8; i += 1024) { crow[2 * i] = 0x10100000u; crow[2 * i + 1] = 0x1010u; }
        for (int i = tid; i < n_rt * 16; i += 1024) rowmode[i] = i < n_coef ? -(i + 1) : 0;
        if (tid < d) z_dev[tid] = ix.z[tid];
    }
    if (do_z && tid < 64) {
        if (tid <= d) Ac[tid] = tid == 0 ? 1 : 0;
        __builtin_amdgcn_fence(__ATOMIC_RELEASE, "wavefront");
        __builtin_amdgcn_wave_barrier();
        for (int q = 0; q < d; q++) {
            i128 nv = 0;
            const bool act = tid <= q + 1 && tid <= d;
            if (act) nv = (tid > 0 ? Ac[tid - 1] : (i128)0) - (i128)ix.xz[q] * Ac[tid];
            __builtin_amdgcn_fence(__ATOMIC_ACQ_REL, "wavefront");
            __builtin_amdgcn_wave_barrier();
            if (act) Ac[tid] = nv;
            __builtin_amdgcn_fence(__ATOMIC_ACQ_REL, "wavefront");
            __builtin_amdgcn_wave_barrier();
        }
        if (tid < d) {
            const i128 xj = ix.xz[tid];
            i128 cur = 1;
            for (int m = d - 1; m >= 0; m--) {
                if (m < n_coef) ent[(size_t)m * d + tid] = cur;
                if (m > 0) cur = Ac[m] + xj * cur;
            }
        }
    } else if (do_z && tid < 64 + 4 * FS_MAXD + 32) {
        const int j = (tid - 64) >> 2, pq = (tid - 64) & 3;
        if (j < d) {
            uint32_t w[NL];
            fp_set(w, P.one);
            const uint32_t *row = inv + (size_t)ix.z[j] * n * NL;
            for (int q = pq; q < d; q += 4) {
                if (q == j) continue;
                uint32_t f[NL];
#pragma unroll
                for (int k = 0; k < NL; k++) f[k] = row[(size_t)ix.z[q] * NL + k];
                mont_mul(w, w, f, P);
            }
#pragma unroll
            for (int k = 0; k < NL; k++) part[((size_t)j * 4 + pq) * NL + k] = w[k];
        }
    } else if (do_zc && tid >= 256) {
        for (int e = tid - 256; e < nc * d; e += 1024 - 256) {
            const int i = e / d, j = e - i * d;
            const int64_t xi = ix.xzc[i];
            i128 v = 1;
            for (int q = 0; q < d; q++)
                if (q != j) v *= (i128)(xi - (int64_t)ix.xz[q]);
            ent[(size_t)(n_coef + i) * d + j] = v;
        }
    }
    __syncthreads();
    if (do_z && tid < d) {
        uint32_t a[NL], b[NL], c[NL];
#pragma unroll
        for (int k = 0; k < NL; k++) { a[k] = part[((size_t)tid * 4) * NL + k]; b[k] = part[((size_t)tid * 4 + 1) * NL + k]; }
        mont_mul(c, a, b, P);
#pragma unroll
        for (int k = 0; k < NL; k++) { a[k] = part[((size_t)tid * 4 + 2) * NL + k]; b[k] = part[((size_t)tid * 4 + 3) * NL + k]; }
        mont_mul(a, a, b, P);
        mont_mul(c, c, a, P);
#pragma unroll
        for (int k = 0; k < NL; k++) wj[(size_t)tid * NL + k] = c[k];
    }
    __syncthreads();
    const int row_lo = do_z ? 0 : n_coef, row_hi = do_zc ? n_out : n_coef;
    for (int e = tid + row_lo * d; e < row_hi * d; e += 1024) {
        const int i = e / d, l = e - i * d;
        i128 v = ent[e];
        const bool negv = v < 0;
        int carry = 0;
#pragma unroll
        for (int b = 0; b < 16; b++) {
            int t = (int)((uint32_t)(v >> (8 * b)) & 0xffu) + carry;
            if (t > 127) { t -= 256; carry = 1; } else carry = 0;
            a8[fs_digit_addr(i, l, b, nkb)] = (uint8_t)(int8_t)t;
        }
        if (carry != (negv ? 1 : 0) && status) atomicOr(status, FS_OVERFLOW);
    }
    for (int i = tid + row_lo; i < row_hi; i += 1024) fs_row_constant(P, cs, ent + (size_t)i * d, d, crow + (size_t)i * 16);
    if (do_zc)
        for (int i = tid; i < nc; i += 1024) rowmode[n_coef + i] = (int32_t)ix.zc[i] + 1;
    if (do_z) {
        for (int e = tid; e < d * NL; e += 1024) {
            const int l = e / NL, q = e - l * NL;
            uint32_t w[NL], two[NL], tq[NL];
#pragma unroll
            for (int k = 0; k < NL; k++) { w[k] = wj[(size_t)l * NL + k]; two[k] = (k == q) ? 1u : 0u; }
            mont_mul(tq, w, two, P);
#pragma unroll
            for (int k = 0; k < NL; k++) KT[((size_t)l * NL + q) * NL + k] = tq[k];
        }
    }
}

__device__ __forceinline__ void fs_cand_body(uint8_t *fc_lds, const FpParams<9> &P, int n, const uint16_t *__restrict__ xs, const FsIdx &ix, int d, const FsConsts &cs,
                                             uint8_t *__restrict__ cand, uint32_t *__restrict__ cand_crow, int32_t *__restrict__ status) {
    i128 *ent = reinterpret_cast<i128 *>(fc_lds);
    const int tid = threadIdx.x, nkb = (d + 7) / 8;
    const size_t row_bytes = (size_t)nkb * 8 * 16;
    for (size_t i = tid; i < (size_t)n * row_bytes / 16; i += 1024) reinterpret_cast<uint4 *>(cand)[i] = make_uint4(0, 0, 0, 0);
    for (int e = tid; e < n * d; e += 1024) {
        const int i = e / d, j = e - i * d;
        const int64_t xi = xs[i];
        i128 v = 1;
        for (int q = 0; q < d; q++)
            if (q != j) v *= (i128)(xi - (int64_t)ix.xz[q]);
        ent[e] = v;
    }
    __syncthreads();
    for (int e = tid; e < n * d; e += 1024) {
        const int i = e / d, l = e - i * d;
        const i128 v = ent[e];
        const bool negv = v < 0;
        const int kb = l >> 3, gg = (l & 7) >> 1, el = l & 1;
        int carry = 0;
#pragma unroll
        for (int b = 0; b < 16; b++) {
            int t = (int)((uint32_t)(v >> (8 * b)) & 0xffu) + carry;
            if (t > 127) { t -= 256; carry = 1; } else carry = 0;
            const int grp = b >> 3, r7 = 7 - (b & 7), hi = r7 >> 2, bi = r7 & 3;
            cand[(size_t)i * row_bytes + (size_t)(((kb * 2 + grp) * 4 + gg) * 16) + 4 * (2 * hi + el) + bi] = (uint8_t)(int8_t)t;
        }
        if (carry != (negv ? 1 : 0) && status) atomicOr(status, FS_OVERFLOW);
    }
    for (int i = tid; i < n; i += 1024) fs_row_constant(P, cs, ent + (size_t)i * d, d, cand_crow + (size_t)i * 16);
}

__global__ void __launch_bounds__(1024) k_fs_build(const FpParams<9> P, const uint32_t *__restrict__ inv, int n, const FsIdx ix, int d, int nc, int n_coef,
                                                   int flags, const FsConsts cs, uint8_t *__restrict__ a8, uint32_t *__restrict__ crow, uint32_t *__restrict__ KT,
                                                   int32_t *__restrict__ rowmode, int32_t *__restrict__ z_dev, int32_t *__restrict__ status) {
    extern __shared__ __attribute__((aligned(16))) uint8_t fs_b_lds[];
    fs_build_body(fs_b_lds, P, inv, n, ix, d, nc, n_coef, flags, cs, a8, crow, KT, rowmode, z_dev, status);
}

__global__ void __launch_bounds__(1024) k_fs_cand(const FpParams<9> P, int n, const uint16_t *__restrict__ xs, const FsIdx ix, int d, const FsConsts cs,
                                                  uint8_t *__restrict__ cand, uint32_t *__restrict__ cand_crow, int32_t *__restrict__ status) {
    extern __shared__ __attribute__((aligned(16))) uint8_t fs_c_lds[];
    fs_cand_body(fs_c_lds, P, n, xs, ix, d, cs, cand, cand_crow, status);
}

__global__ void __launch_bounds__(1024) k_fs_build_z_cand(const FpParams<9> P, const uint32_t *__restrict__ inv, int n, const uint16_t *__restrict__ xs, const FsIdx ix, int d, int nc,
                                                          int n_coef, const FsConsts cs, uint8_t *__restrict__ a8, uint32_t *__restrict__ crow, uint32_t *__restrict__ KT,
                                                          int32_t *__restrict__ rowmode, int32_t *__restrict__ z_dev, uint8_t *__restrict__ cand, uint32_t *__restrict__ cand_crow,
                                                          int32_t *__restrict__ status) {
    extern __shared__ __attribute__((aligned(16))) uint8_t fs_zc_lds[];
    if (blockIdx.x == 0) fs_build_body(fs_zc_lds, P, inv, n, ix, d, nc, n_coef, FS_BUILD_Z, cs, a8, crow, KT, rowmode, z_dev, status);
    else fs_cand_body(fs_zc_lds, P, n, xs, ix, d, cs, cand, cand_crow, status);
}

static int fs_num_cus() {
    static int n = 0;
    if (!n) {
        int dev = 0;
        (void)hipGetDevice(&dev);
        if (hipDeviceGetAttribute(&n, hipDeviceAttributeMultiprocessorCount, dev) != hipSuccess || n <= 0) n = 256;
    }
    return n;
}

int fs_layout(hb_ctx *ctx, const PointTable *pt, int d, int nc, int n_coef, FsLayout *L) {
    if (ctx->n_limbs != 4 || !pt || !pt->usable || !pt->small) return HB_ERR_UNSUPPORTED;
    if (d < 4 || d > 22 || nc < 0 || nc > FS_MAXC || n_coef < 1 || n_coef > d) return HB_ERR_UNSUPPORTED;
    if (env_hook(ENV_NO_MFMA) || env_hook(ENV_NO_FUSED_SMALL) || env_hook(ENV_NO_QUICK) || !prescale_params(ctx)) return HB_ERR_UNSUPPORTED;
    if ((int64_t)d * 16 * 128 * 128 > MM8_BIAS) return HB_ERR_UNSUPPORTED;
    std::vector<uint16_t> xs(pt->xs);
    std::sort(xs.begin(), xs.end());
    double bits_n = 0.0, bits_p = 0.0;
    for (int k = 0; k < d - 1 && k < (int)xs.size(); k++) bits_n += log2(1.0 + xs[xs.size() - 1 - k]);
    const int R = xs.empty() ? 0 : xs.back() - xs.front();
    for (int k = 0; k < d - 1; k++) { const int dist = R - k / 2; if (dist < 1) break; bits_p += log2((double)dist); }
    if (bits_n > 124.5 || bits_p > 124.5) return HB_ERR_UNSUPPORTED;
    L->n = pt->n; L->d = d; L->nc = nc; L->n_coef = n_coef; L->n_out = n_coef + nc;
    L->nkb = (d + 7) / 8; L->n_rt = (L->n_out + 15) / 16;
    if (fs_lds_bytes(L->n_rt, L->nkb) > FS_LDS_LIMIT) return HB_ERR_UNSUPPORTED;
    auto al = [](size_t v) { return (v + 255) & ~(size_t)255; };
    L->o_a8 = 0;
    L->o_crow = al((size_t)L->n_rt * L->nkb * 2 * 64 * 16);
    L->o_kt = L->o_crow + al((size_t)L->n_rt * 16 * 16 * 4);
    L->o_mode = L->o_kt + al((size_t)d * 81 * 4);
    L->o_z = L->o_mode + al((size_t)L->n_rt * 16 * 4);
    L->need = L->o_z + al((size_t)FS_MAXD * 4);
    L->o_cand = L->o_cand_crow = 0;
    if (pt->n <= FS_CAND_MAXN && nc > 0) {
        L->o_cand = L->need;
        L->o_cand_crow = L->o_cand + al((size_t)pt->n * L->nkb * 8 * 16);
        L->need = L->o_cand_crow + al((size_t)pt->n * 16 * 4);
    }
    return HB_OK;
}

int fs_build(hb_ctx *ctx, const PointTable *pt, const int32_t *z, const int32_t *zc, const FsLayout &L, uint8_t *base, int flags, int32_t *status_dev, hipStream_t s) {
    const int n = L.n, d = L.d, nc = L.nc;
    FsIdx ix;
    memset(&ix, 0, sizeof ix);
    uint64_t seen[4] = {0, 0, 0, 0};
    std::vector<uint8_t> seen_big;
    if (n > 256) seen_big.assign((size_t)n, 0);
    auto mark = [&](int v) -> bool {
        if (v < 0 || v >= n) return false;
        if (n > 256) { if (seen_big[v]) return false; seen_big[v] = 1; return true; }
        if (seen[v >> 6] >> (v & 63) & 1) return false;
        seen[v >> 6] |= 1ull << (v & 63);
        return true;
    };
    for (int i = 0; i < d; i++) { if (!mark(z[i])) return fail(ctx, HB_ERR_BAD_ARG, "fused decode: arrival indices"); ix.z[i] = (uint16_t)z[i]; ix.xz[i] = pt->xs[z[i]]; }
    if (flags & FS_BUILD_ZC)
        for (int j = 0; j < nc; j++) { if (!mark(zc[j])) return fail(ctx, HB_ERR_BAD_ARG, "fused decode: compared indices"); ix.zc[j] = (uint16_t)zc[j]; ix.xzc[j] = pt->xs[zc[j]]; }
    const Mm8Shared *sh = nullptr;
    int rc = mm8_shared(ctx, &sh, s); if (rc) return rc;
    FsConsts cs;
    memcpy(cs.c80r, sh->c80r, sizeof cs.c80r);
    memcpy(cs.biasmod, sh->biasmod, sizeof cs.biasmod);
    const size_t lds = ((size_t)L.n_out * d + d + 1) * 16 + ((size_t)d * 9 + (size_t)d * 4 * 9) * 4;
    k_fs_build<<<1, 1024, lds, s>>>(ctx->pw, pt->inv, n, ix, d, nc, L.n_coef, flags, cs, base + L.o_a8, (uint32_t *)(base + L.o_crow), (uint32_t *)(base + L.o_kt),
                                    (int32_t *)(base + L.o_mode), (int32_t *)(base + L.o_z), status_dev);
    HB_LAUNCH_CHECK(ctx);
    return HB_OK;
}

int fs_build_cand(hb_ctx *ctx, PointTable *pt, const int32_t *z, const FsLayout &L, uint8_t *base, int32_t *status_dev, hipStream_t s, bool with_z) {
    if (!L.o_cand) return fail(ctx, HB_ERR_BAD_ARG, "fused decode: no candidate store in this layout");
    if (!pt->xs_dev) {
        HB_HIP(ctx, hipMalloc(&pt->xs_dev, (size_t)pt->n * 2));
        int rc = upload_table(ctx, pt->xs_dev, pt->xs.data(), (size_t)pt->n * 2, s);
        if (rc) { (void)hipFree(pt->xs_dev); pt->xs_dev = nullptr; return rc; }
    }
    FsIdx ix;
    memset(&ix, 0, sizeof ix);
    uint64_t seen[2] = {0, 0};
    for (int i = 0; i < L.d; i++) {
        const int v = z[i];
        if (v < 0 || v >= pt->n || (seen[v >> 6] >> (v & 63) & 1)) return fail(ctx, HB_ERR_BAD_ARG, "fused decode: arrival indices");
        seen[v >> 6] |= 1ull << (v & 63);
        ix.z[i] = (uint16_t)v; ix.xz[i] = pt->xs[v];
    }
    const Mm8Shared *sh = nullptr;
    int rc = mm8_shared(ctx, &sh, s); if (rc) return rc;
    FsConsts cs;
    memcpy(cs.c80r, sh->c80r, sizeof cs.c80r);
    memcpy(cs.biasmod, sh->biasmod, sizeof cs.biasmod);
    if (with_z) {
        const size_t lds_b = ((size_t)L.n_out * L.d + L.d + 1) * 16 + ((size_t)L.d * 9 + (size_t)L.d * 4 * 9) * 4, lds_c = (size_t)pt->n * L.d * 16;
        k_fs_build_z_cand<<<2, 1024, std::max(lds_b, lds_c), s>>>(ctx->pw, pt->inv, pt->n, pt->xs_dev, ix, L.d, L.nc, L.n_coef, cs, base + L.o_a8, (uint32_t *)(base + L.o_crow),
                                                                  (uint32_t *)(base + L.o_kt), (int32_t *)(base + L.o_mode), (int32_t *)(base + L.o_z), base + L.o_cand,
                                                                  (uint32_t *)(base + L.o_cand_crow), status_dev);
        HB_LAUNCH_CHECK(ctx);
        return HB_OK;
    }
    k_fs_cand<<<1, 1024, (size_t)pt->n * L.d * 16, s>>>(ctx->pw, pt->n, pt->xs_dev, ix, L.d, cs, base + L.o_cand, (uint32_t *)(base + L.o_cand_crow), status_dev);
    HB_LAUNCH_CHECK(ctx);
    return HB_OK;
}

static FsSplit fs_split(int d, int n_rt, int n_out) {
    constexpr int PASS = 95, RAGGED = 70, TERM = 36;
    FsSplit sp;
    int load[FS_WAVES];
    const int n_pairs = FS_TPW * n_rt;
    const bool ragged = n_out - 16 * (n_rt - 1) <= 8;
    for (int w = 0; w < FS_WAVES; w++) {
        sp.terms[w] = 0;
        load[w] = 0;
        for (int pidx = w; pidx < n_pairs; pidx += FS_WAVES) {
            const int tl = n_rt == 2 ? (pidx >> 1) : pidx / n_rt;
            const int rt = n_rt == 2 ? ((pidx ^ (pidx >> 2)) & 1) : pidx - tl * n_rt;
            load[w] += (ragged && rt == n_rt - 1) ? RAGGED : PASS;
        }
    }
    for (int l = 0; l < d; l++) {
        int best = FS_WAVES - 1;
        for (int w = FS_WAVES - 2; w >= 0; w--)
            if (load[w] < load[best]) best = w;
        sp.terms[best] |= 1u << l;
        load[best] += TERM;
    }
    return sp;
}

int fs_launch(hb_ctx *ctx, const FsLayout &L, const uint8_t *base, const uint32_t *cols, hb_view cv, uint32_t *out, hb_view ov, int64_t out_count,
              int32_t *mismatch_dev, int32_t *first_bad_dev, uint32_t *bad_map_dev, int64_t C, hipStream_t s, const FsDone *done_p, const int32_t *pick_zc) {
    FsDone done;
    memset(&done, 0, sizeof done);
    if (done_p) done = *done_p;
    FsPick pick;
    memset(&pick, 0, sizeof pick);
    if (pick_zc) {
        if (!L.o_cand) return fail(ctx, HB_ERR_BAD_ARG, "fused decode: no candidate store to pick from");
        pick.cand = (const uint4 *)(base + L.o_cand); pick.cand_crow = (const uint32_t *)(base + L.o_cand_crow);
        pick.n_coef = L.n_coef; pick.nc = L.nc;
        for (int j = 0; j < L.nc; j++) pick.zc[j] = (uint16_t)pick_zc[j];
    }
    if (C <= 0) return HB_OK;
    const Mm8Shared *sh = nullptr;
    int rc = mm8_shared(ctx, &sh, s); if (rc) return rc;
    const int64_t n_units = (C + 63) / 64;
    int64_t blocks = fs_num_cus();
    if (blocks > n_units) blocks = n_units;
    blocks = mm8_trimmed_grid(n_units, blocks);
    const size_t lds = fs_lds_bytes(L.n_rt, L.nkb);
    const FsSplit split = fs_split(L.d, L.n_rt, L.n_out);
#define FS_LAUNCH(NKB)                                                                                                                     \
    do {                                                                                                                                   \
        static std::atomic<unsigned long long> attr_done{0};                                                                                                        \
        if (!((attr_done.load() >> (ctx->device & 63)) & 1ull)) { HB_HIP(ctx, hipFuncSetAttribute(reinterpret_cast<const void *>(k_mm8f<NKB>), hipFuncAttributeMaxDynamicSharedMemorySize, 160 * 1024)); attr_done.fetch_or(1ull << (ctx->device & 63)); } \
        k_mm8f<NKB><<<dim3((unsigned)blocks), dim3(64 * FS_WAVES), lds, s>>>((const int4 *)(base + L.o_a8), (const uint32_t *)(base + L.o_crow), sh->fold_dev,        \
            (const uint32_t *)(base + L.o_kt), ctx->psc, cols, cv.stride_c, cv.stride_l, (const int32_t *)(base + L.o_z), INT64_MAX, L.d, (const int32_t *)(base + L.o_mode), \
            out, ov.stride_c, ov.stride_l, out_count, mismatch_dev, first_bad_dev, bad_map_dev, L.n_out, L.n_rt, C, n_units, sh->bp, done, pick, split); \
    } while (0)
    switch (L.nkb) {
        case 1: FS_LAUNCH(1); break;
        case 2: FS_LAUNCH(2); break;
        case 3: FS_LAUNCH(3); break;
        default: return fail(ctx, HB_ERR_UNSUPPORTED, "fused decode: more than 24 terms");
    }
#undef FS_LAUNCH
    HB_LAUNCH_CHECK(ctx);
    return HB_OK;
}

}

#ifdef HB_MM8_TIMING
extern "C" int hb_debug_fs_timing(unsigned long long *out, int count) {
    return hipMemcpyFromSymbol(out, HIP_SYMBOL(hb::g_fs_t), sizeof(unsigned long long) * (size_t)count) == hipSuccess ? 0 : 1;
}
#endif
```

### honeybadgermpc_amd/csrc/hb_mm8.hpp

```cpp
#pragma once
#include "hb_common.hpp"

namespace hb {

typedef int v4i __attribute__((ext_vector_type(4)));

constexpr int MM8_NC = 47;
constexpr int MM8_CW = 13;
constexpr int MM8_FOLD_ROW = 272;
constexpr int MM8_FOLD_Q = 8 * MM8_FOLD_ROW / 16;
constexpr int MM8_BIAS = 5800000;

struct BarrettParams {
    uint32_t pneg[8];
    uint32_t c384[8];
    uint32_t mu;
};

struct Mm8Matrix {
    int n_out, d, nkb, n_rt;
    bool skip01;
    int4 *a8;
    uint32_t *crow;
    uint32_t *zero;
    BarrettParams bp;
};

struct Mm8Shared {
    BarrettParams bp;
    uint32_t c80r[9], biasmod[9];
    uint8_t fold_host[MM8_FOLD_Q * 16];
    v4i *fold_dev;
};
int mm8_shared(hb_ctx *ctx, const Mm8Shared **out, hipStream_t s);
int64_t mm8_trimmed_grid(int64_t n_units, int64_t blocks);
void mm8_shared_free(hb_ctx *ctx);

}
```

### honeybadgermpc_amd/csrc/hb_open.hip

```cpp
#include "hb_common.hpp"

using namespace hb;

struct hb_open_plan {
    hb_ctx *ctx;
    int n, d, n_check;
    int64_t max_B, max_C;
    FastMatrix *V;
    FastMatrix *Vinv;
    Mm8Matrix *V8;
    Mm8Matrix *Vzc8;
    int32_t *zc_dev, *ones_dev;
    std::vector<int32_t> zc;
    std::vector<int32_t> z;
    std::vector<uint64_t> x;
    Mm8Matrix *Vinv8;
    uint32_t *scaled_pk;
    int use_v8;
    int use_fused;
    int fused_pending;
    int decode_calls;
    int32_t *z_dev;
    int32_t *mask_dev;
    uint32_t *in_dg;
    uint32_t *coef_dg;
    int32_t *mismatch_dev;
    int validate_arrived_only;
    int ntt_order;
    uint32_t *tw;
    uint32_t *coef_pk;
    hb_matrix *Winv;
    const Mm8wMatrix *Winv8;
    hb_matrix *Vw;
    const Mm8wMatrix *Vw8;
    Mm8wMatrix *F1, *F2;
    int32_t *fmap1, *fmap2;
    uint8_t *q1, *q2;
    QuickLayout l1, l2;
    const Mm8wShared *qsh;
    uint8_t *fs1, *fs2;
    FsLayout fl1, fl2;
    Mv64Matrix *nv_enc, *nv_f1, *nv_f2;
};

static void build_quick_wide(hb_open_plan *pl, hipStream_t s) {
    hb_ctx *ctx = pl->ctx;
    if (pl->q1 || env_hook(ENV_NO_QUICK_PLAN)) return;
    QuickLayout a, b;
    const int n = pl->n, d = pl->d, n_check = pl->n_check;
    if (quick_layout(ctx, n, d, n_check, 1, &a) == HB_OK && quick_layout(ctx, n, d, n_check, d, &b) == HB_OK) {
        uint8_t *b1 = nullptr, *b2 = nullptr;
        const Mm8wShared *sh = nullptr;
        int qrc = HB_OK;
        if (hipMalloc(&b1, a.need) != hipSuccess || hipMalloc(&b2, b.need) != hipSuccess) qrc = HB_ERR_HIP;
        const int32_t *zcp = n_check > 0 ? pl->zc.data() : pl->z.data();
        if (!qrc) qrc = quick_build(ctx, pl->x.data(), pl->z.data(), zcp, a, b1, &sh, s);
        if (!qrc) qrc = quick_build(ctx, pl->x.data(), pl->z.data(), zcp, b, b2, &sh, s);
        if (!qrc) { pl->q1 = b1; pl->q2 = b2; pl->l1 = a; pl->l2 = b; pl->qsh = sh; pl->fused_pending = 0; }
        else { if (b1) (void)hipFree(b1); if (b2) (void)hipFree(b2); }
    }
    ctx->err.clear();
}

static void build_fused_small(hb_open_plan *pl, hipStream_t s) {
    hb_ctx *ctx = pl->ctx;
    if (pl->fs1 || env_hook(ENV_NO_QUICK_PLAN) || env_hook(ENV_NO_QUICK)) return;
    PointTable *pt = nullptr;
    FsLayout a, b;
    if (point_table(ctx, pl->x.data(), pl->n, &pt, s) == HB_OK && fs_layout(ctx, pt, pl->d, pl->n_check, 1, &a) == HB_OK &&
        fs_layout(ctx, pt, pl->d, pl->n_check, pl->d, &b) == HB_OK) {
        uint8_t *b1 = nullptr, *b2 = nullptr;
        int qrc = HB_OK;
        if (hipMalloc(&b1, a.need) != hipSuccess || hipMalloc(&b2, b.need) != hipSuccess) qrc = HB_ERR_HIP;
        const int32_t *zcp = pl->n_check > 0 ? pl->zc.data() : pl->z.data();
        if (!qrc) qrc = fs_build(ctx, pt, pl->z.data(), zcp, a, b1, FS_BUILD_Z | FS_BUILD_ZC, pl->mismatch_dev, s);
        if (!qrc) qrc = fs_build(ctx, pt, pl->z.data(), zcp, b, b2, FS_BUILD_Z | FS_BUILD_ZC, pl->mismatch_dev, s);
        if (!qrc) { pl->fs1 = b1; pl->fs2 = b2; pl->fl1 = a; pl->fl2 = b; pl->fused_pending = 0; }
        else { if (b1) (void)hipFree(b1); if (b2) (void)hipFree(b2); }
    }
    ctx->err.clear();
}

static int valu_planes(hb_open_plan *pl) {
    if (pl->in_dg && pl->coef_dg) return HB_OK;
    hb_ctx *ctx = pl->ctx;
    const size_t bytes = (size_t)pl->max_C * pl->d * ctx->nl() * 4;
    if (!pl->in_dg && hipMalloc(&pl->in_dg, bytes) != hipSuccess) return fail(ctx, HB_ERR_HIP, "open plan: hipMalloc(in_dg)");
    if (!pl->coef_dg && hipMalloc(&pl->coef_dg, bytes) != hipSuccess) return fail(ctx, HB_ERR_HIP, "open plan: hipMalloc(coef_dg)");
    return HB_OK;
}

static int build_fused(hb_open_plan *pl, const uint64_t *x_host, hipStream_t s) {
    hb_ctx *ctx = pl->ctx;
    const int d = pl->d, nc = pl->n_check, L = ctx->n_limbs;
    std::vector<uint64_t> W((size_t)d * d * L), P((size_t)nc * d * L);
    int rc = hb_matrix_to_host(ctx, pl->Winv, W.data(), s);
    if (rc) return rc;
    if (nc > 0) {
        std::vector<uint64_t> xzc((size_t)nc * L);
        for (int j = 0; j < nc; j++) memcpy(&xzc[(size_t)j * L], x_host + (size_t)pl->zc[j] * L, (size_t)L * 8);
        hb_matrix *Vzc = nullptr;
        uint32_t *Wd = nullptr, *Pd = nullptr;
        rc = hb_vand_matrix_create(ctx, xzc.data(), nc, d, &Vzc, s);
        if (!rc) rc = upload_elems(ctx, W.data(), (size_t)d * d, &Wd, s);
        if (!rc && hipMalloc(&Pd, P.size() * 8) != hipSuccess) rc = fail(ctx, HB_ERR_HIP, "fused validate: hipMalloc");
        if (!rc) rc = hb_matvec(ctx, Vzc, (const uint64_t *)Wd, hb_view{1, d}, nullptr, (uint64_t *)Pd, hb_view{1, d}, d, s);
        if (!rc && hipMemcpyAsync(P.data(), Pd, P.size() * 8, hipMemcpyDeviceToHost, s) != hipSuccess) rc = fail(ctx, HB_ERR_HIP, "fused validate: copy");
        if (!rc && hipStreamSynchronize(s) != hipSuccess) rc = fail(ctx, HB_ERR_HIP, "fused validate: sync");
        if (Vzc) matrix_unref(Vzc);
        if (Wd) (void)hipFree(Wd);
        if (Pd) (void)hipFree(Pd);
        if (rc) return rc;
    }
    std::vector<uint64_t> m2((size_t)(d + nc) * d * L), m1((size_t)(1 + nc) * d * L);
    memcpy(m2.data(), W.data(), W.size() * 8);
    memcpy(m1.data(), W.data(), (size_t)d * L * 8);
    if (nc > 0) {
        memcpy(&m2[(size_t)d * d * L], P.data(), P.size() * 8);
        memcpy(&m1[(size_t)d * L], P.data(), P.size() * 8);
    }
    std::vector<int32_t> map2((size_t)d + nc + 1, 0), map1((size_t)1 + nc + 1, 0);
    for (int j = 0; j < nc; j++) { map2[(size_t)d + j] = pl->zc[j] + 1; map1[(size_t)1 + j] = pl->zc[j] + 1; }
    rc = mm8w_from_host(ctx, m2.data(), d + nc, d, &pl->F2, s);
    if (!rc) rc = mm8w_from_host(ctx, m1.data(), 1 + nc, d, &pl->F1, s);
    if (!rc) rc = own_int_array(ctx, map2.data(), (int)map2.size(), &pl->fmap2, s);
    if (!rc) rc = own_int_array(ctx, map1.data(), (int)map1.size(), &pl->fmap1, s);
    if (rc) {
        mm8w_free(pl->F1); mm8w_free(pl->F2); pl->F1 = pl->F2 = nullptr;
        if (pl->fmap1) { (void)hipFree(pl->fmap1); pl->fmap1 = nullptr; }
        if (pl->fmap2) { (void)hipFree(pl->fmap2); pl->fmap2 = nullptr; }
        return rc == HB_ERR_UNSUPPORTED ? HB_OK : rc;
    }
    return HB_OK;
}

static int ensure_fused(hb_open_plan *pl, hipStream_t s) {
    pl->fused_pending = 0;
    if (pl->q1 || pl->F1 || pl->d < 4 || pl->n < 4 || env_hook(ENV_NO_MFMA_DECODE)) return HB_OK;
    hb_ctx *ctx = pl->ctx;
    const int L = ctx->n_limbs;
    if (!pl->Winv) {
        std::vector<uint64_t> xz((size_t)pl->d * L);
        for (int i = 0; i < pl->d; i++) memcpy(&xz[(size_t)i * L], &pl->x[(size_t)pl->z[i] * L], (size_t)L * 8);
        int rc = hb_vand_inverse_create(ctx, xz.data(), pl->d, &pl->Winv, (void *)s);
        if (rc) return rc;
        pl->Winv8 = matrix_wide(ctx, pl->Winv, s);
    }
    return pl->Winv8 ? build_fused(pl, pl->x.data(), s) : HB_OK;
}

extern "C" {

int hb_open_plan_create(hb_ctx *ctx, int n, int d, int use_omega_powers, const uint64_t *x_host,
                        const uint64_t *omega_host, int order, const int32_t *z_host, const int32_t *zc_host,
                        int n_check, int64_t max_B, hb_open_plan **out, void *stream) { HB_API_GUARD(ctx);
    if (!ctx || !out || n <= 0 || d <= 0 || d > n || !x_host || !z_host || max_B < 0) return HB_ERR_BAD_ARG;
    if (n_check < 0 || n_check > n || (n_check > 0 && !zc_host)) return HB_ERR_BAD_ARG;
// ... 296 lines not shown
```

### honeybadgermpc_amd/csrc/hb_quick.hip

```cpp
#include <algorithm>
#include <atomic>
#include <chrono>

#include "hb_common.hpp"

using namespace hb;

namespace hb {

constexpr int QUICK_MAX = 128;
constexpr int QUICK_MAXC = 256;
constexpr int PROBE_MAXN = 256;
constexpr int PROBE_NT = 1024;

struct QuickIdx { uint16_t z[QUICK_MAX], zc[QUICK_MAXC]; };
struct ProbeIdx { uint16_t idx[PROBE_MAXN]; };

template <int NL> __device__ __forceinline__ void ldg(uint32_t (&r)[NL], const uint32_t *p) {
#pragma unroll
    for (int i = 0; i < NL; i++) r[i] = p[i];
}
template <int NL> __device__ __forceinline__ void stg(uint32_t *p, const uint32_t (&r)[NL]) {
#pragma unroll
    for (int i = 0; i < NL; i++) p[i] = r[i];
// ... 1005 lines not shown
    const int frows = (cand && do_z) ? n : nc;
    if (do_z || nc > 0) {
        const int nw = (d + QM_FPB - 1) / QM_FPB, nf = std::max(1, (frows + QM_FPB - 1) / QM_FPB);
        const int nh = L.n_coef == 1 ? nw : ((do_z && d > 40) ? 4 : 1);
        const size_t lds = (size_t)std::max((4 + QM_SEG) * d + 1, d + QM_FSEG * QM_FPB) * 36;
        k_quick_matrix<9><<<nh + nw + nf + (do_z ? 1 : 0), QM_NT, lds, s>>>(ctx->pw, pt->xm, pt->inv, n, ix, d, nc, L.n_coef, wj, full, nraw, (int32_t *)(base + L.o_z),
                                                          (int32_t *)(base + L.o_map), (flags & 3) | (cand && do_z ? 4 : 0), (uint4 *)base, (int)(L.o_wj / 16),
                                                          (uint4 *)(base + L.o_cand), (cand && do_z) ? (int)((L.o_cand_crow - L.o_cand) / 16) : 0,
                                                          nh, nw, nf, pt->pw, pt->S);
    }
    HB_LAUNCH_CHECK(ctx);
    if (cand && do_z) {
        k_quick_fill<<<(unsigned)(L.n_coef + n), QF_NT, 0, s>>>(ctx->pw, pt->inv, n, ix, d, L.n_coef, wj, full, nraw, base + L.o_a8, (uint32_t *)(base + L.o_crow),
                                                               L.tile_rows, L.nkb, rcs, base + L.o_cand, (uint32_t *)(base + L.o_cand_crow), 0);
        HB_LAUNCH_CHECK(ctx);
        return HB_OK;
    }
    if (do_z && do_zc && d <= QF_NT) {
        k_quick_fill<<<(unsigned)L.n_out, QF_NT, 0, s>>>(ctx->pw, pt->inv, n, ix, d, L.n_coef, wj, full, nraw, base + L.o_a8, (uint32_t *)(base + L.o_crow),
                                                        L.tile_rows, L.nkb, rcs, nullptr, nullptr, 1);
        HB_LAUNCH_CHECK(ctx);
        return HB_OK;
    }
    if (row_hi > row_lo) {
        k_quick_image<<<(unsigned)(((row_hi - row_lo) * d + 255) / 256), 256, 0, s>>>(ctx->pw, pt->inv, n, ix, d, nc, L.n_coef, wj, full, nraw, mcan, base + L.o_a8, L.tile_rows, L.nkb, row_lo, row_hi);
        HB_LAUNCH_CHECK(ctx);
        k_quick_rows<<<(unsigned)((row_hi - row_lo + 63) / 64), 64, 0, s>>>(ctx->pw, mcan, row_lo, row_hi, d, rcs, (uint32_t *)(base + L.o_crow), L.tile_rows);
        HB_LAUNCH_CHECK(ctx);
    }
    return HB_OK;
}

int quick_launch(hb_ctx *ctx, const QuickLayout &L, const uint8_t *base, const Mm8wShared *sh, const uint32_t *cols, hb_view cv, uint32_t *out, hb_view ov,
                 int64_t out_count, int n_store, int32_t *mismatch_dev, int32_t *first_bad_dev, int64_t C, hipStream_t s, uint32_t *bad_map_dev, const FsDone *done) {
    const int32_t *fmap = (const int32_t *)(base + L.o_map);
    return launch_mm8w_raw(ctx, L.n_out, L.d, L.tile_rows, (const void *)(base + L.o_a8), (const uint32_t *)(base + L.o_crow), sh,
                           cols, cv, (const int32_t *)(base + L.o_z), INT64_MAX, out, ov, out_count,
                           L.nc > 0 ? fmap : nullptr, mismatch_dev, C, s, cols, cv, n_store, L.nc > 0 ? first_bad_dev : nullptr, L.nc > 0 ? bad_map_dev : nullptr,
                           L.nc > 0 ? done : nullptr);
}

}

extern "C" {

int hb_quick_interp_check(hb_ctx *ctx, const uint64_t *x_host, int n, const int32_t *z, int d, const int32_t *zc, int nc,
                          const uint64_t *cols_dev, int64_t C, int64_t chunk_lo, int64_t chunk_hi, uint64_t *coeffs_dev, int32_t *status_dev, void *stream) {
    return hb_quick_interp_check_map(ctx, x_host, n, z, d, zc, nc, cols_dev, C, chunk_lo, chunk_hi, coeffs_dev, status_dev, nullptr, stream);
}

int hb_quick_interp_check_map(hb_ctx *ctx, const uint64_t *x_host, int n, const int32_t *z, int d, const int32_t *zc, int nc,
                              const uint64_t *cols_dev, int64_t C, int64_t chunk_lo, int64_t chunk_hi, uint64_t *coeffs_dev, int32_t *status_dev,
                              uint32_t *bad_map_dev, void *stream) { HB_API_GUARD(ctx);
    if (!ctx || !x_host || !z || n < 1 || d < 1 || d > n || nc < 0 || (nc > 0 && !zc) || C < 0 || chunk_lo < 0 || chunk_hi > C || chunk_lo > chunk_hi) return HB_ERR_BAD_ARG;
    if (chunk_hi == chunk_lo) return HB_OK;
    if (!cols_dev || (nc > 0 && !status_dev)) return HB_ERR_BAD_ARG;
    hipStream_t s = (hipStream_t)stream;
    cache_trim(ctx);
    auto take_slot = [&](size_t need, hb_ctx::QuickSlot **out) -> int {
        if (ctx->qslots.empty()) ctx->qslots.resize(4);
        hb_ctx::QuickSlot &sl = ctx->qslots[ctx->qnext++ % ctx->qslots.size()];
        if (sl.ev) HB_HIP(ctx, hipEventSynchronize((hipEvent_t)sl.ev));
        else { hipEvent_t ev; HB_HIP(ctx, hipEventCreateWithFlags(&ev, hipEventDisableTiming)); sl.ev = ev; }
        if (sl.cap < need) {
            if (sl.buf) HB_HIP(ctx, hipFree(sl.buf));
            sl.buf = nullptr; sl.cap = 0;
            HB_HIP(ctx, hipMalloc(&sl.buf, need));
            sl.cap = need;
        }
        *out = &sl;
        return HB_OK;
    };
    const int64_t cnt = chunk_hi - chunk_lo;
    const uint32_t *in = (const uint32_t *)cols_dev + (size_t)chunk_lo * 8;
    hb_view pm{1, C}, dv{d, 1};
    if (ctx->n_limbs == 4 && !env_hook(ENV_NO_QUICK)) {
        PointTable *pt = nullptr;
        FsLayout F;
        int rc = point_table(ctx, x_host, n, &pt, s); if (rc) return rc;
        if (fs_layout(ctx, pt, d, nc, coeffs_dev ? d : 1, &F) == HB_OK) {
            hb_ctx::QuickSlot *sl = nullptr;
            rc = take_slot(F.need, &sl); if (rc) return rc;
            uint8_t *base = static_cast<uint8_t *>(sl->buf);
            rc = fs_build(ctx, pt, z, zc, F, base, FS_BUILD_Z | FS_BUILD_ZC, status_dev, s); if (rc) return rc;
            uint32_t *out = coeffs_dev ? (uint32_t *)coeffs_dev + (size_t)chunk_lo * d * 8 : nullptr;
            rc = fs_launch(ctx, F, base, in, pm, out, dv, coeffs_dev ? cnt * (int64_t)d : 0, status_dev, (nc > 0 && status_dev) ? status_dev + 1 : nullptr,
                           nc > 0 ? bad_map_dev : nullptr, cnt, s);
            if (rc) return rc;
            HB_HIP(ctx, hipEventRecord((hipEvent_t)sl->ev, s));
            return HB_OK;
        }
    }
    QuickLayout L;
    int rc = quick_layout(ctx, n, d, nc, coeffs_dev ? d : 1, &L); if (rc) return rc;
    hb_ctx::QuickSlot *slp = nullptr;
    rc = take_slot(L.need, &slp); if (rc) return rc;
    hb_ctx::QuickSlot &sl = *slp;
    uint8_t *base = static_cast<uint8_t *>(sl.buf);
    const Mm8wShared *sh = nullptr;
    rc = quick_build(ctx, x_host, z, zc, L, base, &sh, s); if (rc) return rc;
    uint32_t *out = coeffs_dev ? (uint32_t *)coeffs_dev + (size_t)chunk_lo * d * 8 : (uint32_t *)(base + L.o_mcan);
    rc = quick_launch(ctx, L, base, sh, in, pm, out, dv, coeffs_dev ? cnt * (int64_t)d : 0, coeffs_dev ? d : 0, status_dev, status_dev ? status_dev + 1 : nullptr, cnt, s, bad_map_dev);
    if (rc) return rc;
    HB_HIP(ctx, hipEventRecord((hipEvent_t)sl.ev, s));
    return HB_OK;
}

}

__global__ void k_publish_verdict(int32_t *status, FsVerdict *host, int seq) {
    fs_publish_verdict(status, status + 1, nullptr, host, seq);
}

static hipError_t ctx_side_stream(hb_ctx *ctx, hipStream_t *out) {
    if (!ctx->side_stream) {
        int lo_prio = 0, hi_prio = 0;
        (void)hipDeviceGetStreamPriorityRange(&lo_prio, &hi_prio);
        hipStream_t ss = nullptr;
        const hipError_t e = hipStreamCreateWithPriority(&ss, hipStreamNonBlocking, hi_prio);
        if (e != hipSuccess) return e;
        ctx->side_stream = ss;
    }
    *out = (hipStream_t)ctx->side_stream;
    return hipSuccess;
}
extern "C" int hb_side_stream(hb_ctx *ctx, void **stream) { HB_API_GUARD(ctx);
    if (!ctx || !stream) return HB_ERR_BAD_ARG;
    hipStream_t ss = nullptr;
    HB_HIP(ctx, ctx_side_stream(ctx, &ss));
    *stream = ss;
    return HB_OK;
}

struct hb_quick_dec {
    hb_ctx *ctx;
    int n;
    PointTable *pt;
    bool wide;
    QuickLayout Q;
    const Mm8wShared *qsh;
    std::vector<uint64_t> x;
    FsLayout L;
    uint8_t *buf;
    size_t cap;
    int32_t *status;
    FsVerdict *res_host, *res_dev;
    int seq;
    bool prepared;
    std::vector<int32_t> z;
    hipStream_t bstream;
    hipEvent_t built, launched;
    bool launch_open;
    hipStream_t launch_stream;
    bool beside;
    bool built_beside;
};

namespace hb {
int quick_dec_supported(hb_quick_dec *qd, int d, int nc, int n_coef) { HB_API_GUARD((qd ? qd->ctx : nullptr));
    if (!qd || d < 1 || d > qd->n || nc < 0 || n_coef < 1 || n_coef > d) return HB_ERR_BAD_ARG;
    FsLayout L;
    if (fs_layout(qd->ctx, qd->pt, d, nc, n_coef, &L) == HB_OK) return HB_OK;
    QuickLayout Q;
    return quick_layout(qd->ctx, qd->n, d, nc, n_coef, &Q);
}
}
// ... 427 lines not shown
```

### include/hbmpc_hip_debug.h

```cpp
#ifndef HBMPC_HIP_DEBUG_H
#define HBMPC_HIP_DEBUG_H

#include "hbmpc_hip.h"

#ifdef __cplusplus
extern "C" {
#endif

int hb_debug_mm8_create(hb_ctx *ctx, const uint64_t *x_host, int n, int d, void **out);
int hb_debug_mm8_apply(hb_ctx *ctx, void *mat, const void *in_dev, int64_t in_sc, int64_t in_sl, int64_t in_count,
                       void *out_dev, int64_t out_sc, int64_t out_sl, int64_t out_count, int64_t n_chunks,
                       const int32_t *check_mask_dev, int32_t *mismatch_dev);
int hb_debug_occupancy(int n_in, int nl, int *mv3, int *dc);
void hb_debug_reload_env(void);
void hb_debug_pm_slab_bytes(int64_t bytes);
void hb_debug_rf_stats(int64_t *out);
void hb_debug_rf_profile(int on);
void hb_debug_mat_split(int mode);
int hb_debug_matvec_route(hb_ctx *ctx, const hb_matrix *m, int64_t C, int32_t *out);


#ifdef __cplusplus
}
#endif
#endif
```

Before: 8.529 billion.

## Pack ragged last row tile of fused decode into half-width MFMA phases

Adds a packed mode to the fused mm8 decode kernel. When the last 16-row tile is sparsely filled, two output rows share one accumulator column set: remainder rows are merged, and rows with small points are placed as singles, using new generated asm phases with a single A-buffer group and a halved bias. The goal is to cut the MFMA and LDS work spent on padding rows of the ragged tile. In exchange it adds slot remapping, extra bias constants, a new template dimension, and a tighter bias bound that limits when packing applies.

```diff
diff --git a/honeybadgermpc_amd/_capi.py b/honeybadgermpc_amd/_capi.py
--- a/honeybadgermpc_amd/_capi.py
+++ b/honeybadgermpc_amd/_capi.py
@@ -207,6 +207,10 @@
     "hb_debug_rf_profile": (None, [_i]),
     "hb_debug_mat_split": (None, [_i]),
     "hb_debug_matvec_route": (_i, [_vp, _vp, _i64, _vp]),
+    "hb_debug_fs_pack_rows": (_i, [_i, _i, _i, _vp, _vp]),
+    "hb_debug_fs_pack_points": (_i, [_vp, _i, _i, _i, _vp, _vp]),
+    "hb_debug_fs_slot": (_i, [_i, _i, _vp, _i, _i, _vp]),
+    "hb_debug_fs_last_pack": (_i, []),
 }
 
 _lib = None
diff --git a/honeybadgermpc_amd/csrc/gen_mm8.py b/honeybadgermpc_amd/csrc/gen_mm8.py
--- a/honeybadgermpc_amd/csrc/gen_mm8.py
+++ b/honeybadgermpc_amd/csrc/gen_mm8.py
@@ -28,14 +28,22 @@
     return sorted(c for rho in HALF_RHOS[half] for c in cols_of(rho))
 
 
-def lds_loads(kb, xs_op, as_op):
+NCP = 39
+
+
+def packed_columns(half):
+    return sorted(4 * q + rho + 7 for rho in HALF_RHOS[half] for q in windows(rho))
+
+
+def lds_loads(kb, xs_op, as_op, packed=False):
     a0, a1 = ABUF[kb & 1]
     out = []
     for e in (0, 1):
         for h in (0, 1):
             out.append(f"ds_read_b128 v[{XB + 8 * e + 4 * h}:{XB + 8 * e + 4 * h + 3}], {xs_op} offset:{((kb * 2 + e) * 2 + h) * 1024}")
     out.append(f"ds_read_b128 v[{a0}:{a0 + 3}], {as_op} offset:{(kb * 2) * 1024}")
-    out.append(f"ds_read_b128 v[{a1}:{a1 + 3}], {as_op} offset:{(kb * 2 + 1) * 1024}")
+    if not packed:
+        out.append(f"ds_read_b128 v[{a1}:{a1 + 3}], {as_op} offset:{(kb * 2 + 1) * 1024}")
     return out
 
 
@@ -57,9 +65,10 @@
     return out
 
 
-def asm_half(half, nkb, skip=False):
+def asm_half(half, nkb, skip=False, packed=False):
     assert not skip or nkb >= 2
-    cols = half_columns(half)
+    assert not (skip and packed)
+    cols = packed_columns(half) if packed else half_columns(half)
     pos = {c: i for i, c in enumerate(cols)}
     ncol = len(cols)
     xs_op, as_op, bias = f"%{ncol}", f"%{ncol + 1}", f"%{ncol + 2}"
@@ -68,7 +77,7 @@
         for k in (-2, 8):
             for e in (0, 1):
                 L.append(f"v_mov_b32 v{f(s, k, e)}, 0")
-    L += lds_loads(0, xs_op, as_op)[:(5 if skip else 6)]
+    L += lds_loads(0, xs_op, as_op, packed)[:(5 if skip else 6)]
     groups = [(kb, rho) for kb in range(nkb) for rho in HALF_RHOS[half]]
 
     def prep(gi):
@@ -100,7 +109,7 @@
         for q in windows(rho):
             r = f(s, q, 0)
             assert r % 2 == 0
-            for grp in (0, 1):
+            for grp in ((0,) if packed else (0, 1)):
                 if skip and kb == 0 and grp == 1:
                     continue
                 c = 4 * q + rho + 7 + 8 * grp
@@ -118,7 +127,7 @@
         nxt = gi + 1 < len(groups)
         kb, rho = groups[gi]
         if rho == HALF_RHOS[half][0] and kb + 1 < nkb:
-            L += lds_loads(kb + 1, xs_op, as_op)
+            L += lds_loads(kb + 1, xs_op, as_op, packed)
         L += interleave(mfmas(gi), prep(gi + 1) if nxt else [])
         if nxt:
             L.append("s_nop 0")
@@ -150,6 +159,24 @@
             out.append(f'            : {clob}, "memory");')
             out.append("    }")
             out.append("};")
+    assert packed_columns(0) == [c for c in range(NCP) if c % 4 in (0, 3)] and packed_columns(1) == [c for c in range(NCP) if c % 4 in (1, 2)]
+    out.append("// packed phases: accumulator i of a half is the virtual column (one per window) of the same two lists cut at 38")
+    out.append("template <int NKB, int HALF> struct Mm8PhasePacked;")
+    for nkb in range(1, MAXKB + 1):
+        for half in range(2):
+            lines, ncol = asm_half(half, nkb, packed=True)
+            assert sum("v_mfma" in ln for ln in lines) == len(windows(HALF_RHOS[half][0]) + windows(HALF_RHOS[half][1])) * nkb
+            out.append(f"template <> struct Mm8PhasePacked<{nkb}, {half}> {{")
+            out.append("    static __device__ __forceinline__ void run(v4i (&acc)[20], uint32_t xs_addr, uint32_t as_addr, v4i biasv) {")
+            out.append("        asm volatile(")
+            for ln in lines:
+                out.append(f'            "{ln}\\n\\t"')
+            outs = ", ".join(f'"=&v"(acc[{i}])' for i in range(ncol))
+            out.append(f"            : {outs}")
+            out.append('            : "v"(xs_addr), "v"(as_addr), "v"(biasv)')
+            out.append(f'            : {clob}, "memory");')
+            out.append("    }")
+            out.append("};")
     return "\n".join(out) + "\n"
 
 
diff --git a/honeybadgermpc_amd/csrc/hb_common.hpp b/honeybadgermpc_amd/csrc/hb_common.hpp
--- a/honeybadgermpc_amd/csrc/hb_common.hpp
+++ b/honeybadgermpc_amd/csrc/hb_common.hpp
@@ -101,6 +101,7 @@
     ENV_MM8W_TILE16,
     ENV_MM8_NO_SKIP,
     ENV_NO_EVAL_FEW,
+    ENV_NO_FUSED_PACK,
     ENV_NO_FUSED_SMALL,
     ENV_NO_FUSED_VALIDATE,
     ENV_NO_MFMA,
@@ -352,10 +353,13 @@
 struct FsLayout {
     int n, d, nc, n_coef, n_out, n_rt, nkb;
     size_t o_a8, o_crow, o_kt, o_mode, o_z, o_cand, o_cand_crow, need;
+    int pk_nm, pk_ns;
+    uint8_t pk_single[8];
 };
 constexpr int FS_BUILD_Z = 1, FS_BUILD_ZC = 2;
 int fs_layout(hb_ctx *ctx, const PointTable *pt, int d, int nc, int n_coef, FsLayout *L);
 int fs_build(hb_ctx *ctx, const PointTable *pt, const int32_t *z, const int32_t *zc, const FsLayout &L, uint8_t *base, int flags, int32_t *status_dev, hipStream_t s);
+bool fs_pack(const PointTable *pt, const int32_t *z, FsLayout *L);
 int fs_launch(hb_ctx *ctx, const FsLayout &L, const uint8_t *base, const uint32_t *cols, hb_view cv, uint32_t *out, hb_view ov, int64_t out_count,
               int32_t *mismatch_dev, int32_t *first_bad_dev, uint32_t *bad_map_dev, int64_t C, hipStream_t s, const FsDone *done = nullptr,
               const int32_t *pick_zc = nullptr);
diff --git a/honeybadgermpc_amd/csrc/hb_core.hip b/honeybadgermpc_amd/csrc/hb_core.hip
--- a/honeybadgermpc_amd/csrc/hb_core.hip
+++ b/honeybadgermpc_amd/csrc/hb_core.hip
@@ -448,7 +448,7 @@
 
 
 namespace hb {
-static const char *const ENV_NAMES[ENV_COUNT] = {"HB_CACHE_CAP", "HB_GAO_PAIR", "HB_MM8W_FLAT", "HB_MM8W_RQ", "HB_MM8W_TILE16", "HB_MM8_NO_SKIP", "HB_NO_EVAL_FEW", "HB_NO_FUSED_SMALL", "HB_NO_FUSED_VALIDATE", "HB_NO_MFMA", "HB_NO_MFMA_DECODE", "HB_NO_MFMA_WIDE", "HB_NO_NARROW_FAST", "HB_NO_QUICK", "HB_NO_QUICK_PLAN", "HB_NTT_STAGE_LOOP", "HB_PROBE_WGS", "HB_QUICK_NO_CAND", "HB_UPLOAD_MODE", "HB_WB_NO_GAO", "HB_WB_NO_UNIFORM"};
+static const char *const ENV_NAMES[ENV_COUNT] = {"HB_CACHE_CAP", "HB_GAO_PAIR", "HB_MM8W_FLAT", "HB_MM8W_RQ", "HB_MM8W_TILE16", "HB_MM8_NO_SKIP", "HB_NO_EVAL_FEW", "HB_NO_FUSED_PACK", "HB_NO_FUSED_SMALL", "HB_NO_FUSED_VALIDATE", "HB_NO_MFMA", "HB_NO_MFMA_DECODE", "HB_NO_MFMA_WIDE", "HB_NO_NARROW_FAST", "HB_NO_QUICK", "HB_NO_QUICK_PLAN", "HB_NTT_STAGE_LOOP", "HB_PROBE_WGS", "HB_QUICK_NO_CAND", "HB_UPLOAD_MODE", "HB_WB_NO_GAO", "HB_WB_NO_UNIFORM"};
 static std::string g_env_val[ENV_COUNT];
 static bool g_env_set[ENV_COUNT];
 static std::once_flag g_env_once;
diff --git a/honeybadgermpc_amd/csrc/hb_mfma.hip b/honeybadgermpc_amd/csrc/hb_mfma.hip
--- a/honeybadgermpc_amd/csrc/hb_mfma.hip
+++ b/honeybadgermpc_amd/csrc/hb_mfma.hip
@@ -423,6 +423,19 @@
     { Big bt(14, 0); for (int c = 0; c < MM8_NC; c++) { Big t(1, (uint32_t)MM8_BIAS); big_add(bt, big_shl(t, 8 * c, 14)); } biasmod = big_divmod(bt, p, nullptr); }
     { Big sft(shift8, shift8 + 8); if (!big_ge(biasmod, sft)) big_add(biasmod, p); big_sub(biasmod, sft); }
     digits9(biasmod, sh->biasmod);
+    for (int merged = 0; merged < 2; merged++) {
+        Big bt(14, 0);
+        for (int c = 0; c < MM8_NCP; c++) {
+            Big t(1, (uint32_t)MM8_BIAS_PACK);
+            big_add(bt, big_shl(t, 8 * c, 14));
+            if (merged) big_add(bt, big_shl(t, 8 * (c + 8), 14));
+        }
+        Big bm = big_divmod(bt, p, nullptr);
+        Big sft(shift8, shift8 + 8);
+        if (!big_ge(bm, sft)) big_add(bm, p);
+        big_sub(bm, sft);
+        digits9(bm, merged ? sh->biasmod_pm : sh->biasmod_ps);
+    }
     {
         Big c80(8, 0x80808080u);
         Big r261(9, 0); r261[8] = 1u << 5;
diff --git a/honeybadgermpc_amd/csrc/hb_mfma_fused.hip b/honeybadgermpc_amd/csrc/hb_mfma_fused.hip
--- a/honeybadgermpc_amd/csrc/hb_mfma_fused.hip
+++ b/honeybadgermpc_amd/csrc/hb_mfma_fused.hip
@@ -23,13 +23,134 @@
 struct FsIdx { uint16_t z[FS_MAXD], xz[FS_MAXD], zc[FS_MAXC], xzc[FS_MAXC]; };
 struct FsPick { const uint4 *cand; const uint32_t *cand_crow; int n_coef, nc; uint16_t zc[FS_MAXC]; };
 struct FsSplit { uint32_t terms[FS_WAVES]; };
+struct FsPack { int nm, ns; uint8_t single[8]; };
+__host__ __device__ inline int fs_slot(const FsPack &pk, int i, int n_out, int &kind) {
+    kind = 0;
+    if (!(pk.nm | pk.ns)) return i;
+    const int base = 16 * ((n_out + 15) / 16 - 1);
+    int before = 0;
+    for (int k = 0; k < pk.ns; k++) {
+        if (pk.single[k] == i) { kind = 2; return base + 4 + (k & 3) + 8 * (k >> 2); }
+        before += pk.single[k] < i;
+    }
+    const int pos = i - before;
+    if (pos >= base) kind = 1;
+    return pos;
+}
+static bool fs_pack_decide(int d, int n_coef, int nc, const uint8_t *small, FsPack *pk) {
+    memset(pk, 0, sizeof *pk);
+    const int n_out = n_coef + nc, rem = n_out - 16 * ((n_out + 15) / 16 - 1);
+    if ((int64_t)d * 8 * 128 * 128 > MM8_BIAS_PACK) return false;
+    if (rem <= 8) { pk->nm = rem; return true; }
+    if (rem == 16) return false;
+    int ns = 0;
+    for (int i = n_coef - 1; i >= 0 && ns < 8; i--)
+        if (small[i]) pk->single[ns++] = (uint8_t)i;
+    std::reverse(pk->single, pk->single + ns);
+    if (rem - ns > 4) { memset(pk, 0, sizeof *pk); return false; }
+    pk->nm = rem - ns; pk->ns = ns;
+    return true;
+}
 constexpr int FS_CAND_MAXN = 128;
 
 __host__ __device__ inline size_t fs_lds_bytes(int n_rt, int nkb) {
     return ((size_t)n_rt * 64 + (size_t)n_rt * nkb * 2 * 64 + (size_t)2 * FS_TPW * nkb * 4 * 64 + MM8_FOLD_Q) * 16 + (size_t)(32 + 16 * n_rt) * 4;
 }
 
-template <int NKB>
+#define FS_REDUCE(I_, F_, E_, C0_) \
+    do { \
+        const int i = (I_); \
+        const int md = maskl[i]; \
+        const bool live = chunk < n_chunks; \
+        const bool cmp = live && md > 0, st = live && md < 0; \
+        uint32_t ew[8]; \
+        load_words<8>(ew, in_pk + (cmp ? (chunk * in_sc + (int64_t)(md - 1) * in_sl) * 8 : 0)); \
+        uint64_t pw[8]; \
+        { \
+            const uint4 *cr = reinterpret_cast<const uint4 *>(crl + (size_t)i * 16); \
+        _Pragma("unroll") \
+            for (int k = 0; k < 4; k++) { \
+                const uint4 c = cr[k]; \
+                pw[2 * k] = (uint64_t)c.x | ((uint64_t)c.y << 32); \
+                pw[2 * k + 1] = (uint64_t)c.z | ((uint64_t)c.w << 32); \
+            } \
+        } \
+        uint32_t glo[5], ghi[5]; \
+        _Pragma("unroll") \
+        for (int k = 0; k < 12; k++) { \
+            uint64_t gk = (uint64_t)F_(k) * k256 + (k < 7 ? pw[k] : 0ull); \
+            if (k < 11) gk += (uint64_t)E_(k) * k16m; \
+            if (k < 7) pw[k] = gk; \
+            else { glo[k - 7] = (uint32_t)gk; ghi[k - 7] = (uint32_t)(gk >> 32); } \
+        } \
+        pw[0] += (uint64_t)(C0_) * u1; \
+        pw[7] += (uint64_t)glo[0] * u1; \
+        uint32_t hw[5]; \
+        { \
+            unsigned cyw = 0; \
+        _Pragma("unroll") \
+            for (int k = 0; k < 4; k++) hw[k] = __builtin_addc(glo[k + 1], ghi[k], cyw, &cyw); \
+            hw[4] = ghi[4] + cyw; \
+        } \
+        v4i hb; \
+        _Pragma("unroll") \
+        for (int k = 0; k < 4; k++) hb[k] = (int)(hw[k] ^ 0x80808080u); \
+        v4i dcol[8]; \
+        _Pragma("unroll") \
+        for (int eb = 0; eb < 8; eb++) \
+            dcol[eb] = __builtin_amdgcn_mfma_i32_16x16x64_i8(fold_lane[eb * (MM8_FOLD_ROW / 16)], hb, v4i{0, 0, 0, 0}, 0, 0, 0); \
+        _Pragma("unroll") \
+        for (int k = 0; k < 8; k++) pw[k] += (uint64_t)hw[4] * bp.c384[k]; \
+        _Pragma("unroll") \
+        for (int k = 0; k < 8; k++) { \
+            int64_t tt = (int64_t)pw[k] + (int64_t)dcol[k][0] * s1; \
+            tt += (int64_t)dcol[k][1] * s256; \
+            tt += (int64_t)dcol[k][2] * s64k; \
+            tt += (int64_t)dcol[k][3] * s16m; \
+            pw[k] = (uint64_t)tt; \
+        } \
+        const uint64_t tq = pw[7] + (pw[6] >> 32); \
+        const uint32_t qh = (uint32_t)(((uint64_t)(uint32_t)(tq >> 16) * bp.mu) >> 46); \
+        _Pragma("unroll") \
+        for (int k = 0; k < 8; k++) pw[k] += (uint64_t)qh * bp.pneg[k]; \
+        uint32_t ow[8]; \
+        uint32_t top; \
+        { \
+            unsigned cy = 0; \
+            ow[0] = (uint32_t)pw[0]; \
+        _Pragma("unroll") \
+            for (int k = 1; k < 8; k++) ow[k] = __builtin_addc((uint32_t)pw[k], (uint32_t)(pw[k - 1] >> 32), cy, &cy); \
+            top = (uint32_t)(pw[7] >> 32) + cy - qh; \
+        } \
+        if (__builtin_amdgcn_ballot_w64(top != 0 || ow[7] >= ~bp.pneg[7]) != 0) { \
+            uint32_t u[8]; \
+            unsigned cy2 = 0; \
+        _Pragma("unroll") \
+            for (int k = 0; k < 8; k++) u[k] = __builtin_addc(ow[k], bp.pneg[k], cy2, &cy2); \
+            const bool take = cy2 || top; \
+        _Pragma("unroll") \
+            for (int k = 0; k < 8; k++) ow[k] = take ? u[k] : ow[k]; \
+        } \
+        uint32_t diff = 0; \
+        _Pragma("unroll") \
+        for (int k = 0; k < 8; k++) diff |= ew[k] ^ ow[k]; \
+        asm volatile("" : "+v"(diff), "+v"(ow[0]), "+v"(ow[1]), "+v"(ow[2]), "+v"(ow[3]), "+v"(ow[4]), "+v"(ow[5]), "+v"(ow[6]), "+v"(ow[7])); \
+        const unsigned long long bad_lanes = __builtin_amdgcn_ballot_w64(cmp && diff); \
+        if (bad_lanes) { \
+            const uint32_t bits16 = (uint32_t)((bad_lanes | (bad_lanes >> 16) | (bad_lanes >> 32) | (bad_lanes >> 48)) & 0xffffull); \
+            if (lane == 0) { \
+                const int64_t tile_base = chunk - n; \
+                const int32_t cmin = (int32_t)tile_base + __builtin_ctz(bits16); \
+                if (*reinterpret_cast<volatile int32_t *>(mismatch) == 0) atomicOr(mismatch, 1); \
+                if (first_bad && *reinterpret_cast<volatile int32_t *>(first_bad) > cmin) atomicMin(first_bad, cmin); \
+                if (bad_map) atomicOr(bad_map + (tile_base >> 5), bits16 << (tile_base & 31)); \
+            } \
+        } \
+        const int64_t oidx = chunk * out_sc + (int64_t)(-md - 1) * out_sl; \
+        if (st && oidx < out_count) store_words<8>(out_pk + oidx * 8, ow); \
+    } while (0)
+
+template <int NKB, int PK>
 __global__ __launch_bounds__(64 * FS_WAVES, 2) void k_mm8f(const int4 *__restrict__ a8, const uint32_t *__restrict__ crowd, const v4i *__restrict__ foldg,
                                                           const uint32_t *__restrict__ KT, const PrescaleParams PP,
                                                           const uint32_t *__restrict__ in_pk, int64_t in_sc, int64_t in_sl, const int32_t *__restrict__ in_rows,
@@ -38,6 +159,8 @@
                                                           int32_t *__restrict__ mismatch, int32_t *__restrict__ first_bad, uint32_t *__restrict__ bad_map,
                                                           int n_out, int n_rt, int64_t n_chunks, int64_t n_units, BarrettParams bp, const FsDone done, const FsPick pick,
                                                           const FsSplit split) {
+    constexpr bool PACKED = PK != 0;
+    const int n_slots = PACKED ? 16 * n_rt : n_out;
     constexpr int NT = 64 * FS_WAVES, NL = 9, NW = 8;
     extern __shared__ uint4 fs_lds[];
     const int lane = threadIdx.x & 63, wave = __builtin_amdgcn_readfirstlane(threadIdx.x >> 6);
@@ -71,7 +194,7 @@
     }
     uint4 pk_piece = make_uint4(0, 0, 0, 0), pk_crow = make_uint4(0, 0, 0, 0);
     const int pk_e = threadIdx.x;
-    const bool pk_has_piece = pick.cand && pk_e < pick.nc * NKB * 8, pk_has_crow = pick.cand && pk_e < pick.nc * 4;
+    const bool pk_has_piece = !PACKED && pick.cand && pk_e < pick.nc * NKB * 8, pk_has_crow = !PACKED && pick.cand && pk_e < pick.nc * 4;
     if (pk_has_piece) {
         const int j = pk_e / (NKB * 8), pc = pk_e - j * (NKB * 8);
         pk_piece = pick.cand[(size_t)pick.zc[j] * (NKB * 8) + pc];
@@ -81,7 +204,7 @@
         const int tid = threadIdx.x, n_mask = n_rt * 16, n_crow = n_rt * 64, n_img = n_rt * NKB * 2 * 64;
         const int lc = tid < d ? tid : d - 1;
         int32_t rw = in_rows ? in_rows[lc] : lc;
-        int32_t mk = rowmode[tid < n_out ? tid : 0];
+        int32_t mk = rowmode[tid < n_slots ? tid : 0];
         v4i cr = reinterpret_cast<const v4i *>(crowd)[tid < n_crow ? tid : 0];
         v4i fo = foldg[tid < MM8_FOLD_Q ? tid : 0];
         v4i img[3];
@@ -89,13 +212,13 @@
         for (int k = 0; k < 3; k++) img[k] = reinterpret_cast<const v4i *>(a8)[tid + k * NT < n_img ? tid + k * NT : 0];
         asm volatile("" : "+v"(rw), "+v"(mk), "+v"(cr), "+v"(fo), "+v"(img[0]), "+v"(img[1]), "+v"(img[2]));
         if (tid < 32) rowl[tid] = rw;
-        if (tid < n_mask) maskl[tid] = tid < n_out ? mk : 0;
+        if (tid < n_mask) maskl[tid] = tid < n_slots ? mk : 0;
         if (tid < n_crow) reinterpret_cast<v4i *>(fs_lds)[tid] = cr;
         if (tid < MM8_FOLD_Q) foldl[tid] = fo;
 #pragma unroll
         for (int k = 0; k < 3; k++)
             if (tid + k * NT < n_img) reinterpret_cast<v4i *>(abuf)[tid + k * NT] = img[k];
-        for (int i = tid + NT; i < n_mask; i += NT) maskl[i] = i < n_out ? rowmode[i] : 0;
+        for (int i = tid + NT; i < n_mask; i += NT) maskl[i] = i < n_slots ? rowmode[i] : 0;
         for (int i = tid + NT; i < n_crow; i += NT) fs_lds[i] = reinterpret_cast<const uint4 *>(crowd)[i];
         for (int i = tid + 3 * NT; i < n_img; i += NT) abuf[i] = a8[i];
     }
@@ -182,7 +305,7 @@
     };
 
     scale_unit(std::true_type{}, blockIdx.x, xbuf, first_terms);
-    if (pick.cand) {
+    if (!PACKED && pick.cand) {
         __syncthreads();
         auto put = [&](int e, const uint4 &v) {
             const int j = e / (NKB * 8), pc = e - j * (NKB * 8);
@@ -224,9 +347,97 @@
             const int4 *as = abuf + (size_t)rt * NKB * 2 * 64 + lane;
             uint32_t eap[4][11], c0p[4];
             const int rows_here = n_out - 16 * rt < 16 ? n_out - 16 * rt : 16;
-            const int nreg = (rows_here + 3) >> 2;
+            const int nreg = PACKED ? 4 : (rows_here + 3) >> 2;
             const uint32_t xs_addr = (uint32_t)(uintptr_t)(__attribute__((address_space(3))) const void *)xs;
             const uint32_t as_addr = (uint32_t)(uintptr_t)(__attribute__((address_space(3))) const void *)as;
+            if (PACKED && rt == n_rt - 1) {
+                const v4i biaspv = v4i{MM8_BIAS_PACK, MM8_BIAS_PACK, MM8_BIAS_PACK, MM8_BIAS_PACK};
+                auto park_merged = [&](auto rc, const v4i (&acc)[20]) __attribute__((always_inline)) {
+                    constexpr int r = decltype(rc)::value;
+                    c0p[r] = (uint32_t)acc[0][r];
+#pragma unroll
+                    for (int j = 0; j < 11; j++) {
+                        uint32_t lo = 0, hi = 0;
+                        if (j < 9) { lo = (uint32_t)acc[1 + 2 * j][r]; hi = (uint32_t)acc[2 + 2 * j][r]; }
+                        if (j >= 2) { lo += (uint32_t)acc[2 * j - 3][r + 2]; hi += (uint32_t)acc[2 * j - 2][r + 2]; }
+                        if (j == 1) hi += (uint32_t)acc[0][r + 2];
+                        eap[r][j] = lo + (hi << 8);
+                    }
+                };
+                auto park_single = [&](auto rc, const v4i (&acc)[20]) __attribute__((always_inline)) {
+                    constexpr int r = decltype(rc)::value;
+                    c0p[r] = (uint32_t)acc[0][r];
+#pragma unroll
+                    for (int j = 0; j < 11; j++) eap[r][j] = j < 9 ? (uint32_t)acc[1 + 2 * j][r] + ((uint32_t)acc[2 + 2 * j][r] << 8) : 0u;
+                };
+                auto keep = [&](auto rc) __attribute__((always_inline)) {
+                    constexpr int r = decltype(rc)::value;
+                    asm volatile("" ::"v"(c0p[r]), "v"(eap[r][0]), "v"(eap[r][1]), "v"(eap[r][2]), "v"(eap[r][3]), "v"(eap[r][4]), "v"(eap[r][5]),
+                                 "v"(eap[r][6]), "v"(eap[r][7]), "v"(eap[r][8]), "v"(eap[r][9]), "v"(eap[r][10]));
+                    __builtin_amdgcn_sched_barrier(0);
+                };
+                {
+                    v4i acc[20];
+                    asm volatile("" ::: "memory");
+                    __builtin_amdgcn_sched_barrier(0);
+                    __builtin_amdgcn_s_setprio(0);
+                    Mm8PhasePacked<NKB, 0>::run(acc, xs_addr, as_addr, biaspv);
+                    __builtin_amdgcn_s_setprio(2);
+                    __builtin_amdgcn_sched_barrier(0);
+                    FS_T(3);
+                    park_merged(std::integral_constant<int, 0>{}, acc);
+                    keep(std::integral_constant<int, 0>{});
+                    if constexpr (PK == 1) park_merged(std::integral_constant<int, 1>{}, acc);
+                    else park_single(std::integral_constant<int, 1>{}, acc);
+                    keep(std::integral_constant<int, 1>{});
+                    if constexpr (PK == 2) {
+                        park_single(std::integral_constant<int, 3>{}, acc);
+                        keep(std::integral_constant<int, 3>{});
+                    }
+                }
+                {
+                    v4i acc[20];
+                    asm volatile("" ::: "memory");
+                    __builtin_amdgcn_sched_barrier(0);
+                    FS_T(4);
+                    __builtin_amdgcn_s_setprio(0);
+                    Mm8PhasePacked<NKB, 1>::run(acc, xs_addr, as_addr, biaspv);
+                    __builtin_amdgcn_s_setprio(2);
+                    __builtin_amdgcn_sched_barrier(0);
+                    FS_T(5);
+                    auto pair_merged = [&](auto rc, int k) __attribute__((always_inline)) {
+                        constexpr int r = decltype(rc)::value;
+                        uint32_t lo = 0, hi = 0;
+                        if (k < 10) { lo = (uint32_t)acc[2 * k][r]; hi = (uint32_t)acc[2 * k + 1][r]; }
+                        if (k >= 2) { lo += (uint32_t)acc[2 * k - 4][r + 2]; hi += (uint32_t)acc[2 * k - 3][r + 2]; }
+                        return lo + (hi << 8);
+                    };
+                    auto pair_single = [&](auto rc, int k) __attribute__((always_inline)) {
+                        constexpr int r = decltype(rc)::value;
+                        return k < 10 ? (uint32_t)acc[2 * k][r] + ((uint32_t)acc[2 * k + 1][r] << 8) : 0u;
+                    };
+#define FS_FM0(k) pair_merged(std::integral_constant<int, 0>{}, k)
+#define FS_FM1(k) pair_merged(std::integral_constant<int, 1>{}, k)
+#define FS_FS1(k) pair_single(std::integral_constant<int, 1>{}, k)
+#define FS_FS3(k) pair_single(std::integral_constant<int, 3>{}, k)
+#define FS_E0(k) eap[0][k]
+#define FS_E1(k) eap[1][k]
+#define FS_E3(k) eap[3][k]
+                    if constexpr (PK == 2) { FS_REDUCE(16 * rt + 12 + g, FS_FS3, FS_E3, c0p[3]); __builtin_amdgcn_sched_barrier(0); }
+                    FS_REDUCE(16 * rt + g, FS_FM0, FS_E0, c0p[0]);
+                    if constexpr (PK == 1) FS_REDUCE(16 * rt + 4 + g, FS_FM1, FS_E1, c0p[1]);
+                    else FS_REDUCE(16 * rt + 4 + g, FS_FS1, FS_E1, c0p[1]);
+#undef FS_FM0
+#undef FS_FM1
+#undef FS_FS1
+#undef FS_FS3
+#undef FS_E0
+#undef FS_E1
+#undef FS_E3
+                }
+                FS_T(6);
+                continue;
+            }
             {
                 v4i acc[24];
                 asm volatile("" ::: "memory");
@@ -260,96 +471,11 @@
 #pragma unroll
                 for (int reg = 0; reg < 4; reg++) {
                     if (reg >= 2 && reg >= nreg) break;
-                    const int i = 16 * rt + 4 * reg + g;
-                    const int md = maskl[i];
-                    const bool live = chunk < n_chunks;
-                    const bool cmp = live && md > 0, st = live && md < 0;
-                    uint32_t ew[8];
-                    load_words<8>(ew, in_pk + (cmp ? (chunk * in_sc + (int64_t)(md - 1) * in_sl) * 8 : 0));
-                    uint64_t pw[8];
-                    {
-                        const uint4 *cr = reinterpret_cast<const uint4 *>(crl + (size_t)i * 16);
-#pragma unroll
-                        for (int k = 0; k < 4; k++) {
-                            const uint4 c = cr[k];
-                            pw[2 * k] = (uint64_t)c.x | ((uint64_t)c.y << 32);
-                            pw[2 * k + 1] = (uint64_t)c.z | ((uint64_t)c.w << 32);
-                        }
-                    }
-                    uint32_t glo[5], ghi[5];
-#pragma unroll
-                    for (int k = 0; k < 12; k++) {
-                        const uint32_t f = (uint32_t)acc[2 * k][reg] + ((uint32_t)acc[2 * k + 1][reg] << 8);
-                        uint64_t gk = (uint64_t)f * k256 + (k < 7 ? pw[k] : 0ull);
-                        if (k < 11) gk += (uint64_t)eap[reg][k] * k16m;
-                        if (k < 7) pw[k] = gk;
-                        else { glo[k - 7] = (uint32_t)gk; ghi[k - 7] = (uint32_t)(gk >> 32); }
-                    }
-                    pw[0] += (uint64_t)c0p[reg] * u1;
-                    pw[7] += (uint64_t)glo[0] * u1;
-                    uint32_t hw[5];
-                    {
-                        unsigned cyw = 0;
-#pragma unroll
-                        for (int k = 0; k < 4; k++) hw[k] = __builtin_addc(glo[k + 1], ghi[k], cyw, &cyw);
-                        hw[4] = ghi[4] + cyw;
-                    }
-                    v4i hb;
-#pragma unroll
-                    for (int k = 0; k < 4; k++) hb[k] = (int)(hw[k] ^ 0x80808080u);
-                    v4i dcol[8];
-#pragma unroll
-                    for (int eb = 0; eb < 8; eb++)
-                        dcol[eb] = __builtin_amdgcn_mfma_i32_16x16x64_i8(fold_lane[eb * (MM8_FOLD_ROW / 16)], hb, v4i{0, 0, 0, 0}, 0, 0, 0);
-#pragma unroll
-                    for (int k = 0; k < 8; k++) pw[k] += (uint64_t)hw[4] * bp.c384[k];
-#pragma unroll
-                    for (int k = 0; k < 8; k++) {
-                        int64_t tt = (int64_t)pw[k] + (int64_t)dcol[k][0] * s1;
-                        tt += (int64_t)dcol[k][1] * s256;
-                        tt += (int64_t)dcol[k][2] * s64k;
-                        tt += (int64_t)dcol[k][3] * s16m;
-                        pw[k] = (uint64_t)tt;
-                    }
-                    const uint64_t tq = pw[7] + (pw[6] >> 32);
-                    const uint32_t qh = (uint32_t)(((uint64_t)(uint32_t)(tq >> 16) * bp.mu) >> 46);
-#pragma unroll
-                    for (int k = 0; k < 8; k++) pw[k] += (uint64_t)qh * bp.pneg[k];
-                    uint32_t ow[8];
-                    uint32_t top;
-                    {
-                        unsigned cy = 0;
-                        ow[0] = (uint32_t)pw[0];
-#pragma unroll
-                        for (int k = 1; k < 8; k++) ow[k] = __builtin_addc((uint32_t)pw[k], (uint32_t)(pw[k - 1] >> 32), cy, &cy);
-                        top = (uint32_t)(pw[7] >> 32) + cy - qh;
-                    }
-                    if (__builtin_amdgcn_ballot_w64(top != 0 || ow[7] >= ~bp.pneg[7]) != 0) {
-                        uint32_t u[8];
-                        unsigned cy2 = 0;
-#pragma unroll
-                        for (int k = 0; k < 8; k++) u[k] = __builtin_addc(ow[k], bp.pneg[k], cy2, &cy2);
-                        const bool take = cy2 || top;
-#pragma unroll
-                        for (int k = 0; k < 8; k++) ow[k] = take ? u[k] : ow[k];
-                    }
-                    uint32_t diff = 0;
-#pragma unroll
-                    for (int k = 0; k < 8; k++) diff |= ew[k] ^ ow[k];
-                    asm volatile("" : "+v"(diff), "+v"(ow[0]), "+v"(ow[1]), "+v"(ow[2]), "+v"(ow[3]), "+v"(ow[4]), "+v"(ow[5]), "+v"(ow[6]), "+v"(ow[7]));
-                    const unsigned long long bad_lanes = __builtin_amdgcn_ballot_w64(cmp && diff);
-                    if (bad_lanes) {
-                        const uint32_t bits16 = (uint32_t)((bad_lanes | (bad_lanes >> 16) | (bad_lanes >> 32) | (bad_lanes >> 48)) & 0xffffull);
-                        if (lane == 0) {
-                            const int64_t tile_base = chunk - n;
-                            const int32_t cmin = (int32_t)tile_base + __builtin_ctz(bits16);
-                            if (*reinterpret_cast<volatile int32_t *>(mismatch) == 0) atomicOr(mismatch, 1);
-                            if (first_bad && *reinterpret_cast<volatile int32_t *>(first_bad) > cmin) atomicMin(first_bad, cmin);
-                            if (bad_map) atomicOr(bad_map + (tile_base >> 5), bits16 << (tile_base & 31));
-                        }
-                    }
-                    const int64_t oidx = chunk * out_sc + (int64_t)(-md - 1) * out_sl;
-                    if (st && oidx < out_count) store_words<8>(out_pk + oidx * 8, ow);
+#define FS_F(k) ((uint32_t)acc[2 * (k)][reg] + ((uint32_t)acc[2 * (k) + 1][reg] << 8))
+#define FS_E(k) eap[reg][k]
+                    FS_REDUCE(16 * rt + 4 * reg + g, FS_F, FS_E, c0p[reg]);
+#undef FS_F
+#undef FS_E
                     if (reg & 1) __builtin_amdgcn_sched_barrier(0);
                 }
             }
@@ -364,7 +490,7 @@
 
 typedef __int128 i128;
 
-struct FsConsts { uint32_t c80r[9], biasmod[9]; };
+struct FsConsts { uint32_t c80r[9], biasmod[9], biasmod_pm[9], biasmod_ps[9]; };
 constexpr int32_t FS_OVERFLOW = 0x40000000;
 
 __device__ __forceinline__ size_t fs_digit_addr(int i, int l, int b, int nkb) {
@@ -373,7 +499,7 @@
     return ((((size_t)(i / 16) * nkb + l / 8) * 2 + grp) * 64 + (size_t)lane_) * 16 + 4 * (2 * hi + el) + bi;
 }
 
-__device__ __forceinline__ void fs_row_constant(const FpParams<9> &P, const FsConsts &cs, const i128 *row, int d, uint32_t *dst16) {
+__device__ __forceinline__ void fs_row_constant(const FpParams<9> &P, const FsConsts &cs, const i128 *row, int d, uint32_t *dst16, int kind = 0) {
     constexpr int NL = 9, NW = 8;
     uint32_t s5[5] = {0, 0, 0, 0, 0};
     for (int l = 0; l < d; l++) {
@@ -393,7 +519,7 @@
     unpack<NL, NW>(fe, w8);
     if (negs) fp_neg(fe, fe, P);
 #pragma unroll
-    for (int k = 0; k < NL; k++) { k80[k] = cs.c80r[k]; bm[k] = cs.biasmod[k]; }
+    for (int k = 0; k < NL; k++) { k80[k] = cs.c80r[k]; bm[k] = kind == 0 ? cs.biasmod[k] : kind == 1 ? cs.biasmod_pm[k] : cs.biasmod_ps[k]; }
     mont_mul(prod, fe, k80, P);
     fp_sub(corr, prod, bm, P);
     uint32_t cw[NW];
@@ -408,7 +534,7 @@
 
 __device__ __forceinline__ void fs_build_body(uint8_t *fb_lds, const FpParams<9> &P, const uint32_t *__restrict__ inv, int n, const FsIdx &ix, int d, int nc, int n_coef,
                                               int flags, const FsConsts &cs, uint8_t *__restrict__ a8, uint32_t *__restrict__ crow, uint32_t *__restrict__ KT,
-                                              int32_t *__restrict__ rowmode, int32_t *__restrict__ z_dev, int32_t *__restrict__ status) {
+                                              int32_t *__restrict__ rowmode, int32_t *__restrict__ z_dev, int32_t *__restrict__ status, const FsPack &pk) {
     constexpr int NL = 9, NW = 8;
     const int n_out = n_coef + nc, nkb = (d + 7) / 8, n_rt = (n_out + 15) / 16;
     i128 *ent = reinterpret_cast<i128 *>(fb_lds);
@@ -421,7 +547,7 @@
         const size_t img = (size_t)n_rt * nkb * 2 * 64 * 16;
         for (size_t i = tid; i < img / 16; i += 1024) reinterpret_cast<uint4 *>(a8)[i] = make_uint4(0, 0, 0, 0);
         for (int i = tid; i < n_rt * 16 * 8; i += 1024) { crow[2 * i] = 0x10100000u; crow[2 * i + 1] = 0x1010u; }
-        for (int i = tid; i < n_rt * 16; i += 1024) rowmode[i] = i < n_coef ? -(i + 1) : 0;
+        for (int i = tid; i < n_rt * 16; i += 1024) rowmode[i] = 0;
         if (tid < d) z_dev[tid] = ix.z[tid];
     }
     if (do_z && tid < 64) {
@@ -491,18 +617,25 @@
         const int i = e / d, l = e - i * d;
         i128 v = ent[e];
         const bool negv = v < 0;
-        int carry = 0;
+        int carry = 0, kind;
+        const int sl = fs_slot(pk, i, n_out, kind);
+        bool lost = false;
 #pragma unroll
         for (int b = 0; b < 16; b++) {
             int t = (int)((uint32_t)(v >> (8 * b)) & 0xffu) + carry;
             if (t > 127) { t -= 256; carry = 1; } else carry = 0;
-            a8[fs_digit_addr(i, l, b, nkb)] = (uint8_t)(int8_t)t;
-        }
-        if (carry != (negv ? 1 : 0) && status) atomicOr(status, FS_OVERFLOW);
-    }
-    for (int i = tid + row_lo; i < row_hi; i += 1024) fs_row_constant(P, cs, ent + (size_t)i * d, d, crow + (size_t)i * 16);
-    if (do_zc)
-        for (int i = tid; i < nc; i += 1024) rowmode[n_coef + i] = (int32_t)ix.zc[i] + 1;
+            if (kind == 0) a8[fs_digit_addr(sl, l, b, nkb)] = (uint8_t)(int8_t)t;
+            else if (b < 8 || kind == 1) a8[fs_digit_addr(sl + (b < 8 ? 0 : 8), l, b & 7, nkb)] = (uint8_t)(int8_t)t;
+            else lost |= t != 0;
+        }
+        if ((lost || carry != (negv ? 1 : 0)) && status) atomicOr(status, FS_OVERFLOW);
+    }
+    for (int i = tid + row_lo; i < row_hi; i += 1024) {
+        int kind;
+        const int sl = fs_slot(pk, i, n_out, kind);
+        fs_row_constant(P, cs, ent + (size_t)i * d, d, crow + (size_t)sl * 16, kind);
+        rowmode[sl] = i < n_coef ? -(i + 1) : (int32_t)ix.zc[i - n_coef] + 1;
+    }
     if (do_z) {
         for (int e = tid; e < d * NL; e += 1024) {
             const int l = e / NL, q = e - l * NL;
@@ -551,9 +684,9 @@
 
 __global__ void __launch_bounds__(1024) k_fs_build(const FpParams<9> P, const uint32_t *__restrict__ inv, int n, const FsIdx ix, int d, int nc, int n_coef,
                                                    int flags, const FsConsts cs, uint8_t *__restrict__ a8, uint32_t *__restrict__ crow, uint32_t *__restrict__ KT,
-                                                   int32_t *__restrict__ rowmode, int32_t *__restrict__ z_dev, int32_t *__restrict__ status) {
+                                                   int32_t *__restrict__ rowmode, int32_t *__restrict__ z_dev, int32_t *__restrict__ status, const FsPack pk) {
     extern __shared__ __attribute__((aligned(16))) uint8_t fs_b_lds[];
-    fs_build_body(fs_b_lds, P, inv, n, ix, d, nc, n_coef, flags, cs, a8, crow, KT, rowmode, z_dev, status);
+    fs_build_body(fs_b_lds, P, inv, n, ix, d, nc, n_coef, flags, cs, a8, crow, KT, rowmode, z_dev, status, pk);
 }
 
 __global__ void __launch_bounds__(1024) k_fs_cand(const FpParams<9> P, int n, const uint16_t *__restrict__ xs, const FsIdx ix, int d, const FsConsts cs,
@@ -567,7 +700,7 @@
                                                           int32_t *__restrict__ rowmode, int32_t *__restrict__ z_dev, uint8_t *__restrict__ cand, uint32_t *__restrict__ cand_crow,
                                                           int32_t *__restrict__ status) {
     extern __shared__ __attribute__((aligned(16))) uint8_t fs_zc_lds[];
-    if (blockIdx.x == 0) fs_build_body(fs_zc_lds, P, inv, n, ix, d, nc, n_coef, FS_BUILD_Z, cs, a8, crow, KT, rowmode, z_dev, status);
+    if (blockIdx.x == 0) fs_build_body(fs_zc_lds, P, inv, n, ix, d, nc, n_coef, FS_BUILD_Z, cs, a8, crow, KT, rowmode, z_dev, status, FsPack{});
     else fs_cand_body(fs_zc_lds, P, n, xs, ix, d, cs, cand, cand_crow, status);
 }
 
@@ -595,6 +728,8 @@
     if (bits_n > 124.5 || bits_p > 124.5) return HB_ERR_UNSUPPORTED;
     L->n = pt->n; L->d = d; L->nc = nc; L->n_coef = n_coef; L->n_out = n_coef + nc;
     L->nkb = (d + 7) / 8; L->n_rt = (L->n_out + 15) / 16;
+    L->pk_nm = L->pk_ns = 0;
+    memset(L->pk_single, 0, sizeof L->pk_single);
     if (fs_lds_bytes(L->n_rt, L->nkb) > FS_LDS_LIMIT) return HB_ERR_UNSUPPORTED;
     auto al = [](size_t v) { return (v + 255) & ~(size_t)255; };
     L->o_a8 = 0;
@@ -610,6 +745,37 @@
         L->need = L->o_cand_crow + al((size_t)pt->n * 16 * 4);
     }
     return HB_OK;
+}
+
+static void fs_small_rows(const uint16_t *xz, int d, int n_coef, uint8_t *small) {
+    i128 Ac[FS_MAXD + 1];
+    for (int k = 0; k <= d; k++) Ac[k] = k == 0 ? 1 : 0;
+    for (int q = 0; q < d; q++)
+        for (int k = q + 1; k >= 0; k--) Ac[k] = (k > 0 ? Ac[k - 1] : (i128)0) - (i128)xz[q] * Ac[k];
+    for (int m = 0; m < n_coef; m++) small[m] = 1;
+    const i128 lim = (i128)1 << 62;
+    for (int j = 0; j < d; j++) {
+        i128 cur = 1;
+        for (int m = d - 1; m >= 0; m--) {
+            if (m < n_coef && (cur >= lim || cur <= -lim)) small[m] = 0;
+            if (m > 0) cur = Ac[m] + (i128)xz[j] * cur;
+        }
+    }
+}
+
+bool fs_pack(const PointTable *pt, const int32_t *z, FsLayout *L) {
+    L->pk_nm = L->pk_ns = 0;
+    memset(L->pk_single, 0, sizeof L->pk_single);
+    if (env_hook(ENV_NO_FUSED_PACK)) return false;
+    uint16_t xz[FS_MAXD];
+    uint8_t small[FS_MAXD];
+    for (int i = 0; i < L->d; i++) { if (z[i] < 0 || z[i] >= L->n) return false; xz[i] = pt->xs[z[i]]; }
+    fs_small_rows(xz, L->d, L->n_coef, small);
+    FsPack pk;
+    if (!fs_pack_decide(L->d, L->n_coef, L->nc, small, &pk)) return false;
+    L->pk_nm = pk.nm; L->pk_ns = pk.ns;
+    memcpy(L->pk_single, pk.single, sizeof pk.single);
+    return true;
 }
 
 int fs_build(hb_ctx *ctx, const PointTable *pt, const int32_t *z, const int32_t *zc, const FsLayout &L, uint8_t *base, int flags, int32_t *status_dev, hipStream_t s) {
@@ -634,9 +800,18 @@
     FsConsts cs;
     memcpy(cs.c80r, sh->c80r, sizeof cs.c80r);
     memcpy(cs.biasmod, sh->biasmod, sizeof cs.biasmod);
+    memcpy(cs.biasmod_pm, sh->biasmod_pm, sizeof cs.biasmod_pm);
+    memcpy(cs.biasmod_ps, sh->biasmod_ps, sizeof cs.biasmod_ps);
+    FsPack pk;
+    memset(&pk, 0, sizeof pk);
+    if (L.pk_nm) {
+        if (flags != (FS_BUILD_Z | FS_BUILD_ZC)) return fail(ctx, HB_ERR_BAD_ARG, "fused decode: a packed image is built in one piece");
+        pk.nm = L.pk_nm; pk.ns = L.pk_ns;
+        memcpy(pk.single, L.pk_single, sizeof pk.single);
+    }
     const size_t lds = ((size_t)L.n_out * d + d + 1) * 16 + ((size_t)d * 9 + (size_t)d * 4 * 9) * 4;
     k_fs_build<<<1, 1024, lds, s>>>(ctx->pw, pt->inv, n, ix, d, nc, L.n_coef, flags, cs, base + L.o_a8, (uint32_t *)(base + L.o_crow), (uint32_t *)(base + L.o_kt),
-                                    (int32_t *)(base + L.o_mode), (int32_t *)(base + L.o_z), status_dev);
+                                    (int32_t *)(base + L.o_mode), (int32_t *)(base + L.o_z), status_dev, pk);
     HB_LAUNCH_CHECK(ctx);
     return HB_OK;
 }
@@ -662,6 +837,8 @@
     FsConsts cs;
     memcpy(cs.c80r, sh->c80r, sizeof cs.c80r);
     memcpy(cs.biasmod, sh->biasmod, sizeof cs.biasmod);
+    memset(cs.biasmod_pm, 0, sizeof cs.biasmod_pm);
+    memset(cs.biasmod_ps, 0, sizeof cs.biasmod_ps);
     if (with_z) {
         const size_t lds_b = ((size_t)L.n_out * L.d + L.d + 1) * 16 + ((size_t)L.d * 9 + (size_t)L.d * 4 * 9) * 4, lds_c = (size_t)pt->n * L.d * 16;
         k_fs_build_z_cand<<<2, 1024, std::max(lds_b, lds_c), s>>>(ctx->pw, pt->inv, pt->n, pt->xs_dev, ix, L.d, L.nc, L.n_coef, cs, base + L.o_a8, (uint32_t *)(base + L.o_crow),
@@ -675,8 +852,11 @@
     return HB_OK;
 }
 
-static FsSplit fs_split(int d, int n_rt, int n_out) {
-    constexpr int PASS = 95, RAGGED = 70, TERM = 36;
+static std::atomic<int> g_fs_last_pack{-1};
+
+static FsSplit fs_split(int d, int n_rt, int n_out, int pk_nm, int pk_ns) {
+    constexpr int PASS = 95, RAGGED = 70, TERM = 36, PACKED2 = 50, PACKED3 = 55;
+    const int packed = pk_ns ? PACKED3 : PACKED2;
     FsSplit sp;
     int load[FS_WAVES];
     const int n_pairs = FS_TPW * n_rt;
@@ -687,7 +867,7 @@
         for (int pidx = w; pidx < n_pairs; pidx += FS_WAVES) {
             const int tl = n_rt == 2 ? (pidx >> 1) : pidx / n_rt;
             const int rt = n_rt == 2 ? ((pidx ^ (pidx >> 2)) & 1) : pidx - tl * n_rt;
-            load[w] += (ragged && rt == n_rt - 1) ? RAGGED : PASS;
+            load[w] += (pk_nm && rt == n_rt - 1) ? packed : (ragged && rt == n_rt - 1) ? RAGGED : PASS;
         }
     }
     for (int l = 0; l < d; l++) {
@@ -708,6 +888,7 @@
     FsPick pick;
     memset(&pick, 0, sizeof pick);
     if (pick_zc) {
+        if (L.pk_nm) return fail(ctx, HB_ERR_BAD_ARG, "fused decode: a packed image has no rows to pick");
         if (!L.o_cand) return fail(ctx, HB_ERR_BAD_ARG, "fused decode: no candidate store to pick from");
         pick.cand = (const uint4 *)(base + L.o_cand); pick.cand_crow = (const uint32_t *)(base + L.o_cand_crow);
         pick.n_coef = L.n_coef; pick.nc = L.nc;
@@ -721,19 +902,21 @@
     if (blocks > n_units) blocks = n_units;
     blocks = mm8_trimmed_grid(n_units, blocks);
     const size_t lds = fs_lds_bytes(L.n_rt, L.nkb);
-    const FsSplit split = fs_split(L.d, L.n_rt, L.n_out);
-#define FS_LAUNCH(NKB)                                                                                                                     \
+    const FsSplit split = fs_split(L.d, L.n_rt, L.n_out, L.pk_nm, L.pk_ns);
+    const int pack = !L.pk_nm ? 0 : L.pk_ns ? 2 : 1;
+    g_fs_last_pack.store(pack);
+#define FS_LAUNCH(NKB, PK)                                                                                                                   \
     do {                                                                                                                                   \
         static std::atomic<unsigned long long> attr_done{0};                                                                                                        \
-        if (!((attr_done.load() >> (ctx->device & 63)) & 1ull)) { HB_HIP(ctx, hipFuncSetAttribute(reinterpret_cast<const void *>(k_mm8f<NKB>), hipFuncAttributeMaxDynamicSharedMemorySize, 160 * 1024)); attr_done.fetch_or(1ull << (ctx->device & 63)); } \
-        k_mm8f<NKB><<<dim3((unsigned)blocks), dim3(64 * FS_WAVES), lds, s>>>((const int4 *)(base + L.o_a8), (const uint32_t *)(base + L.o_crow), sh->fold_dev,        \
+        if (!((attr_done.load() >> (ctx->device & 63)) & 1ull)) { HB_HIP(ctx, hipFuncSetAttribute(reinterpret_cast<const void *>(k_mm8f<NKB, PK>), hipFuncAttributeMaxDynamicSharedMemorySize, 160 * 1024)); attr_done.fetch_or(1ull << (ctx->device & 63)); } \
+        k_mm8f<NKB, PK><<<dim3((unsigned)blocks), dim3(64 * FS_WAVES), lds, s>>>((const int4 *)(base + L.o_a8), (const uint32_t *)(base + L.o_crow), sh->fold_dev,        \
             (const uint32_t *)(base + L.o_kt), ctx->psc, cols, cv.stride_c, cv.stride_l, (const int32_t *)(base + L.o_z), INT64_MAX, L.d, (const int32_t *)(base + L.o_mode), \
             out, ov.stride_c, ov.stride_l, out_count, mismatch_dev, first_bad_dev, bad_map_dev, L.n_out, L.n_rt, C, n_units, sh->bp, done, pick, split); \
     } while (0)
     switch (L.nkb) {
-        case 1: FS_LAUNCH(1); break;
-        case 2: FS_LAUNCH(2); break;
-        case 3: FS_LAUNCH(3); break;
+        case 1: if (pack == 1) FS_LAUNCH(1, 1); else if (pack == 2) FS_LAUNCH(1, 2); else FS_LAUNCH(1, 0); break;
+        case 2: if (pack == 1) FS_LAUNCH(2, 1); else if (pack == 2) FS_LAUNCH(2, 2); else FS_LAUNCH(2, 0); break;
+        case 3: if (pack == 1) FS_LAUNCH(3, 1); else if (pack == 2) FS_LAUNCH(3, 2); else FS_LAUNCH(3, 0); break;
         default: return fail(ctx, HB_ERR_UNSUPPORTED, "fused decode: more than 24 terms");
     }
 #undef FS_LAUNCH
@@ -743,6 +926,35 @@
 
 }
 
+extern "C" int hb_debug_fs_pack_rows(int d, int n_coef, int nc, const uint8_t *small, int32_t *out) {
+    hb::FsPack pk;
+    const bool ok = d >= 1 && d <= hb::FS_MAXD && n_coef >= 1 && n_coef <= d && nc >= 0 && nc <= hb::FS_MAXC && hb::fs_pack_decide(d, n_coef, nc, small, &pk);
+    if (!ok) memset(&pk, 0, sizeof pk);
+    out[0] = pk.nm; out[1] = pk.ns;
+    for (int k = 0; k < 8; k++) out[2 + k] = pk.single[k];
+    return ok ? 1 : 0;
+}
+extern "C" int hb_debug_fs_pack_points(const int32_t *xz, int d, int n_coef, int nc, int32_t *out, uint8_t *small_out) {
+    if (d < 1 || d > hb::FS_MAXD || n_coef < 1 || n_coef > d) return 0;
+    uint16_t x16[hb::FS_MAXD];
+    uint8_t small[hb::FS_MAXD];
+    for (int i = 0; i < d; i++) x16[i] = (uint16_t)xz[i];
+    hb::fs_small_rows(x16, d, n_coef, small);
+    if (small_out) memcpy(small_out, small, (size_t)n_coef);
+    return hb_debug_fs_pack_rows(d, n_coef, nc, small, out);
+}
+extern "C" int hb_debug_fs_last_pack(void) { return hb::g_fs_last_pack.load(); }
+extern "C" int hb_debug_fs_slot(int nm, int ns, const int32_t *single, int i, int n_out, int32_t *kind) {
+    hb::FsPack pk;
+    memset(&pk, 0, sizeof pk);
+    pk.nm = nm; pk.ns = ns;
+    for (int k = 0; k < 8 && k < ns; k++) pk.single[k] = (uint8_t)single[k];
+    int kd = 0;
+    const int sl = hb::fs_slot(pk, i, n_out, kd);
+    *kind = kd;
+    return sl;
+}
+
 #ifdef HB_MM8_TIMING
 extern "C" int hb_debug_fs_timing(unsigned long long *out, int count) {
     return hipMemcpyFromSymbol(out, HIP_SYMBOL(hb::g_fs_t), sizeof(unsigned long long) * (size_t)count) == hipSuccess ? 0 : 1;
diff --git a/honeybadgermpc_amd/csrc/hb_mm8.hpp b/honeybadgermpc_amd/csrc/hb_mm8.hpp
--- a/honeybadgermpc_amd/csrc/hb_mm8.hpp
+++ b/honeybadgermpc_amd/csrc/hb_mm8.hpp
@@ -10,6 +10,8 @@
 constexpr int MM8_FOLD_ROW = 272;
 constexpr int MM8_FOLD_Q = 8 * MM8_FOLD_ROW / 16;
 constexpr int MM8_BIAS = 5800000;
+constexpr int MM8_NCP = 39;
+constexpr int MM8_BIAS_PACK = MM8_BIAS / 2;
 
 struct BarrettParams {
     uint32_t pneg[8];
@@ -29,6 +31,7 @@
 struct Mm8Shared {
     BarrettParams bp;
     uint32_t c80r[9], biasmod[9];
+    uint32_t biasmod_pm[9], biasmod_ps[9];
     uint8_t fold_host[MM8_FOLD_Q * 16];
     v4i *fold_dev;
 };
diff --git a/honeybadgermpc_amd/csrc/hb_open.hip b/honeybadgermpc_amd/csrc/hb_open.hip
--- a/honeybadgermpc_amd/csrc/hb_open.hip
+++ b/honeybadgermpc_amd/csrc/hb_open.hip
@@ -73,6 +73,7 @@
         int qrc = HB_OK;
         if (hipMalloc(&b1, a.need) != hipSuccess || hipMalloc(&b2, b.need) != hipSuccess) qrc = HB_ERR_HIP;
         const int32_t *zcp = pl->n_check > 0 ? pl->zc.data() : pl->z.data();
+        if (!qrc) { (void)fs_pack(pt, pl->z.data(), &a); (void)fs_pack(pt, pl->z.data(), &b); }
         if (!qrc) qrc = fs_build(ctx, pt, pl->z.data(), zcp, a, b1, FS_BUILD_Z | FS_BUILD_ZC, pl->mismatch_dev, s);
         if (!qrc) qrc = fs_build(ctx, pt, pl->z.data(), zcp, b, b2, FS_BUILD_Z | FS_BUILD_ZC, pl->mismatch_dev, s);
         if (!qrc) { pl->fs1 = b1; pl->fs2 = b2; pl->fl1 = a; pl->fl2 = b; pl->fused_pending = 0; }
diff --git a/honeybadgermpc_amd/csrc/hb_quick.hip b/honeybadgermpc_amd/csrc/hb_quick.hip
--- a/honeybadgermpc_amd/csrc/hb_quick.hip
+++ b/honeybadgermpc_amd/csrc/hb_quick.hip
@@ -1111,6 +1111,7 @@
             hb_ctx::QuickSlot *sl = nullptr;
             rc = take_slot(F.need, &sl); if (rc) return rc;
             uint8_t *base = static_cast<uint8_t *>(sl->buf);
+            (void)fs_pack(pt, z, &F);
             rc = fs_build(ctx, pt, z, zc, F, base, FS_BUILD_Z | FS_BUILD_ZC, status_dev, s); if (rc) return rc;
             uint32_t *out = coeffs_dev ? (uint32_t *)coeffs_dev + (size_t)chunk_lo * d * 8 : nullptr;
             rc = fs_launch(ctx, F, base, in, pm, out, dv, coeffs_dev ? cnt * (int64_t)d : 0, status_dev, (nc > 0 && status_dev) ? status_dev + 1 : nullptr,
diff --git a/include/hbmpc_hip_debug.h b/include/hbmpc_hip_debug.h
--- a/include/hbmpc_hip_debug.h
+++ b/include/hbmpc_hip_debug.h
@@ -18,6 +18,10 @@
 void hb_debug_rf_profile(int on);
 void hb_debug_mat_split(int mode);
 int hb_debug_matvec_route(hb_ctx *ctx, const hb_matrix *m, int64_t C, int32_t *out);
+int hb_debug_fs_pack_rows(int d, int n_coef, int nc, const uint8_t *small, int32_t *out);
+int hb_debug_fs_pack_points(const int32_t *xz, int d, int n_coef, int nc, int32_t *out, uint8_t *small_out);
+int hb_debug_fs_slot(int nm, int ns, const int32_t *single, int i, int n_out, int32_t *kind);
+int hb_debug_fs_last_pack(void);
 
 
 #ifdef __cplusplus
```

After: 8.656 billion (median of 6 runs). 1.01x the previous value.
